# yangyonggit/simple-path-tracer

Measured on AMD Instinct MI355X. Metric: Mrays/sec + Msamples/sec, default scene 1920x1080, 1/2/4/8 MI355X, higher is better.
Workload: dtype f32; 1 GPU; C2: default scene + emitter, 1920x1080, 64 spp, depth 6; scene=default_emitter, width=1920, height=1080, spp=64, max_depth=6, parallelism=tile-sharded x1 (interleaved 32x32 tiles) + RCCL gather to rank 0

## Files before the change

### simple-path-tracer_amd/csrc/kernels_wavefront.hip

```cpp
#include <hip/hip_runtime.h>
#include <hip/hip_ext.h>

#include <algorithm>
#include <cstdlib>
#include <mutex>

#include "cull_prims.h"
#include "sky_split.h"
#include "sptr_internal.h"

#ifndef SPTR_TRACE_WAVES
#define SPTR_TRACE_WAVES 7
#endif
#ifndef SPTR_TRACE_PM_WAVES
#define SPTR_TRACE_PM_WAVES SPTR_TRACE_WAVES
#endif
#ifndef SPTR_TRACE_WP_WAVES
#define SPTR_TRACE_WP_WAVES SPTR_TRACE_WAVES
#endif
#ifndef SPTR_TRACE4_WAVES
#define SPTR_TRACE4_WAVES 7
#endif
#ifndef SPTR_SHADE_WAVES
#define SPTR_SHADE_WAVES 5
// ... 690 lines not shown
  float tn = __builtin_huge_valf();
  uint32_t nxt = 0u, nh = 0u;
#pragma unroll
  for (int k = 0; k < 4; ++k) {
    const bool better = (kAny && kAnyHitFar) ? t[k] > tn : t[k] < tn;
    const bool take = hc[k] & ((kn == 4) | better);
    tn = take ? t[k] : tn;
    kn = take ? k : kn;
    nxt = take ? ln[k] : nxt;
    nh += hc[k] ? 1u : 0u;
  }
  const bool descend = kn < 4;
  if (sp + 3 < N) {
    int pos = sp;
#pragma unroll
    for (int k = 3; k >= 0; --k) {
      stack.lds[pos * kBlock] = ln[k];
      pos += (hc[k] & (k != kn)) ? 1 : 0;
    }
  } else {
    if (sp + (int)nh - 1 > kStack) vc.stack_overflow = 1u;
    int pos = sp;
#pragma unroll
    for (int k = 3; k >= 0; --k)
      if (hc[k] && k != kn && pos < kStack) stack.put(pos++, ln[k]);
  }
  const int spd = sp + (int)nh - 1;
  wk.hit = wk.hit | lhit;
  wk.cur = descend ? nxt : popv;
  wk.sp = descend ? (spd < kStack ? spd : kStack) : ps;
  return (kAny && lhit) || (!descend && sp == 0);
}
template <bool kAny, bool kCount, int N>
__device__ __forceinline__ bool wide_walk_bf(WideWalk& wk, TravStack<N>& stack, const WideNode* nodes,
                                             const uint32_t* prim_ref, const float4* tris, const float4* sph,
                                             const Ray& r, float tnear, float& tfar, uint32_t& ref, Visits& vc, int steps) {
  for (int it = 0; it < steps; ++it)
    if (walk_step_bf<kAny, kCount>(wk, stack, nodes, prim_ref, tris, sph, r, tnear, tfar, ref, vc)) return true;
  return false;
}
template <bool kAny, bool kCount, int kKind = kWalkU, int N>
__device__ __forceinline__ bool wide_walk(WideWalk& wk, TravStack<N>& stack, const WideNode* nodes, const uint4* top,
                                          uint32_t ntop, const uint32_t* prim_ref, const float4* tris, const float4* sph,
                                          const Ray& r, float tnear, float& tfar, uint32_t& ref, Visits& vc, int steps) {
  if constexpr (kKind == kWalkBranchFree)
    return wide_walk_bf<kAny, kCount>(wk, stack, nodes, prim_ref, tris, sph, r, tnear, tfar, ref, vc, steps);
  else if constexpr (kKind == kWalkUnified)
    return wide_walk_u<kAny, kCount>(wk, stack, nodes, top, ntop, prim_ref, tris, sph, r, tnear, tfar, ref, vc, steps);
  else
    return wide_walk_inl<kAny, kCount>(wk, stack, nodes, top, ntop, prim_ref, tris, sph, r, tnear, tfar, ref, vc, steps);
}
template <bool kAny, bool kCount>
__device__ __forceinline__ bool wide_start(WideWalk& wk, uint32_t root, const uint32_t* prim_ref, const float4* tris,
                                           const float4* sph, const Ray& r, float tnear, float& tfar, uint32_t& ref,
                                           Visits& vc) {
  wk.cur = root;
  wk.sp = 0;
  wk.hit = false;
  if (root == kNoHit) return true;
  if (root & kLeafBit) {
    wk.hit = leaf_test<kAny, kCount>(root, prim_ref, tris, sph, r, tnear, tfar, ref, vc);
    return true;
  }
  return false;
}
template <bool kAny, bool kCount, int N>
__device__ __forceinline__ bool traverse_wide(const WideNode* nodes, const uint32_t* prim_ref, const float4* tris,
                                              const float4* sph, uint32_t root, const Ray& r, float tnear, float& tfar,
                                              uint32_t& ref, Visits& vc, LdsStackN<N>& ls) {
  WideWalk wk;
  if (wide_start<kAny, kCount>(wk, root, prim_ref, tris, sph, r, tnear, tfar, ref, vc)) return wk.hit;
  TravStack<N> stack;
  stack.lds = &ls.e[0][threadIdx.x];
  (void)wide_walk<kAny, kCount>(wk, stack, nodes, nullptr, 0u, prim_ref, tris, sph, r, tnear, tfar, ref, vc, 0x7FFFFFFF);
  return wk.hit;
}

struct Staged {
  const BvhNode* nodes;
  const WideNode* nodes4;
  const uint32_t* prim_ref;
  const float4* tris;
  const float4* sph;
};
template <bool kLds>
__device__ __forceinline__ Staged stage_scene(const SceneView& sv, float4* lds) {
  Staged s{sv.nodes, sv.nodes4, sv.prim_ref, sv.tris, sv.sph};
  if (kLds) {
    const bool w4 = sv.width == (uint32_t)kWide;
    const uint32_t nn = (w4 ? sv.num_nodes4 * (uint32_t)sizeof(WideNode) : sv.num_nodes * (uint32_t)sizeof(BvhNode)) / 16u,
                   nt = sv.num_tris * 3u, ns = sv.num_sph;
    const uint32_t np = (sv.num_tris + sv.num_sph + 3u) / 4u;
    const float4* gn = w4 ? reinterpret_cast<const float4*>(sv.nodes4) : reinterpret_cast<const float4*>(sv.nodes);
    const float4* gp = reinterpret_cast<const float4*>(sv.prim_ref);
    for (uint32_t i = threadIdx.x; i < nn; i += blockDim.x) lds[i] = gn[i];
    for (uint32_t i = threadIdx.x; i < nt; i += blockDim.x) lds[nn + i] = sv.tris[i];
    for (uint32_t i = threadIdx.x; i < ns; i += blockDim.x) lds[nn + nt + i] = sv.sph[i];
    for (uint32_t i = threadIdx.x; i < np; i += blockDim.x) lds[nn + nt + ns + i] = gp[i];
    __syncthreads();
    s.nodes = reinterpret_cast<const BvhNode*>(lds);
    s.nodes4 = reinterpret_cast<const WideNode*>(lds);
    s.tris = lds + nn;
    s.sph = lds + nn + nt;
    s.prim_ref = reinterpret_cast<const uint32_t*>(lds + nn + nt + ns);
  }
  return s;
}

__device__ __forceinline__ const uint4* stage_top(const SceneView& sv, float4* dst) {
  const uint32_t n = sv.num_top4 * (uint32_t)(sizeof(WideNode) / 16);
  const uint4* g = reinterpret_cast<const uint4*>(sv.nodes4);
  uint4* d = reinterpret_cast<uint4*>(dst);
  for (uint32_t i = threadIdx.x; i < n; i += blockDim.x) d[i] = g[i];
  return d;
}
__device__ __forceinline__ uint32_t top_lds_offset(const SceneView& sv, bool lds, bool primary, uint32_t nseg) {
  return (lds ? sv.lds_bytes / 16u : 0u) + (primary ? 0u : (4u * (nseg + 1u) + 15u) / 16u);
}

template <bool kW4, bool kAny, bool kCount, int N>
__device__ __forceinline__ bool traverse_w(const Staged& sc, const SceneView& sv, const Ray& r, float tnear, float& tfar,
                                           uint32_t& ref, Visits& vc, LdsStackN<N>& ls) {
  if (kW4) return traverse_wide<kAny, kCount>(sc.nodes4, sc.prim_ref, sc.tris, sc.sph, sv.root4, r, tnear, tfar, ref, vc, ls);
  return traverse<kAny, kCount>(sc.nodes, sc.prim_ref, sc.tris, sc.sph, sv.root, r, tnear, tfar, ref, vc, ls);
}

constexpr uint32_t kEntryFieldBits = 13, kEntryFieldMask = (1u << kEntryFieldBits) - 1u;
template <bool kW4, bool kCount, int N>
__device__ __forceinline__ bool traverse_w_from(const Staged& sc, const SceneView& sv, uint32_t root, const Ray& r,
                                                float& tfar, uint32_t& ref, Visits& vc, LdsStackN<N>& ls) {
  if constexpr (kW4) {
    return traverse_wide<false, kCount>(sc.nodes4, sc.prim_ref, sc.tris, sc.sph, sv.root4, r, 0.0f, tfar, ref, vc, ls);
  } else {
    if (root & kLeafBit) {
      if (root == sv.root) return leaf_test<false, kCount>(root, sc.prim_ref, sc.tris, sc.sph, r, 0.0f, tfar, ref, vc);
      asm volatile("" : "+v"(root));
      const float4* nd = reinterpret_cast<const float4*>(sc.nodes + ((root >> 18) & kEntryFieldMask));
      const uint32_t right = (root >> 17) & 1u;
      const float4 xy = nd[right];
      const float2 z = reinterpret_cast<const float2*>(nd + 2)[right];
      if (kCount) ++vc.nodes;
      float tent;
      if (!slab(xy.x, xy.y, xy.z, xy.w, z.x, z.y, r, 0.0f, tfar, tent)) return false;
      const uint32_t range = kLeafBit | (((root >> 4) & kEntryFieldMask) << kLeafCountBits) | (root & kLeafRangeMask);
      return leaf_test<false, kCount>(range, sc.prim_ref, sc.tris, sc.sph, r, 0.0f, tfar, ref, vc);
    }
    return traverse<false, kCount>(sc.nodes, sc.prim_ref, sc.tris, sc.sph, root, r, 0.0f, tfar, ref, vc, ls);
  }
}

template <bool kW4, bool kAny, bool kCount, int N>
__device__ __forceinline__ bool traverse_w_top(const Staged& sc, const SceneView& sv, const uint4* top, uint32_t ntop,
                                               const Ray& r, float tnear, float& tfar, uint32_t& ref, Visits& vc,
                                               LdsStackN<N>& ls) {
  if constexpr (kW4) {
    WideWalk wk;
    if (wide_start<kAny, kCount>(wk, sv.root4, sc.prim_ref, sc.tris, sc.sph, r, tnear, tfar, ref, vc)) return wk.hit;
    TravStack<N> stack;
    stack.lds = &ls.e[0][threadIdx.x];
    (void)wide_walk<kAny, kCount>(wk, stack, sc.nodes4, top, ntop, sc.prim_ref, sc.tris, sc.sph, r, tnear, tfar, ref, vc,
                                  0x7FFFFFFF);
    return wk.hit;
  }
  return traverse<kAny, kCount>(sc.nodes, sc.prim_ref, sc.tris, sc.sph, sv.root, r, tnear, tfar, ref, vc, ls);
}

__device__ __forceinline__ uint32_t stat_depth(int depth) { return depth < kStatDepths - 1 ? (uint32_t)depth : kStatDepths - 1u; }
__device__ __forceinline__ void hist_ray(uint32_t* s_hist, uint32_t visits) {
  const uint32_t b = visits ? (uint32_t)(32 - __clz(visits)) : 0u;
  atomicAdd(&s_hist[b < (uint32_t)kHistBins ? b : kHistBins - 1u], 1u);
}
__device__ __forceinline__ void hist_init(uint32_t* s_hist) {
  if (threadIdx.x < (uint32_t)kHistBins) s_hist[threadIdx.x] = 0u;
}
__device__ __forceinline__ void hist_flush(const uint32_t* s_hist, unsigned long long* tot, int base) {
  __syncthreads();
  if (threadIdx.x < (uint32_t)kHistBins && s_hist[threadIdx.x]) atomicAdd(&tot[base + threadIdx.x], (unsigned long long)s_hist[threadIdx.x]);
}
__device__ __forceinline__ void flush_depth_nodes(const Visits& vc, unsigned long long* tot, int depth) {
  unsigned long long a = vc.nodes;
  for (int off = 32; off > 0; off >>= 1) a += __shfl_xor(a, off);
  if (lane_id() == 0) atomicAdd(&tot[kTotNodesD + stat_depth(depth)], a);
}

__device__ __forceinline__ void report_stack(const Visits& vc, unsigned long long* tot) {
  if (__ballot(vc.stack_overflow != 0u) && lane_id() == 0u) tot[kTotStackOverflow] = 1ull;
}
// ... 890 lines not shown
        ref = kNoHit;
        if (kCount) v0 = culled ? ~0u : vc.nodes;
        done = walk_start<false, kCount, kW4>(wk, sc, culled ? kNoHit : (kW4 ? sv.root4 : sv.root), r, 0.0f, tfar, ref,
                                              vc);
        have = true;
      }
    }
    if (__ballot(have) == 0ull) {
      if (!more) break;
      continue;
    }
    if (have && !done)
      done = walk_steps<false, kCount, kW4, kKind>(wk, stack, sc, top, ntop, r, 0.0f, tfar, ref, vc,
                                                                          kDynSteps);
    if (!kCount && w.strag_lanes != 0u && drained && (uint32_t)depth < kStragBounces) {
      const unsigned long long act = __ballot(have && !done);
      if (act != 0ull && (uint32_t)__popcll(act) <= w.strag_lanes && have && !done) {
        const uint32_t slot = atomicAdd(&w.work[kWorkStrag + (uint32_t)depth * 32u], 1u);
        if (slot < w.strag_cap) {
          float4* rec = w.strag + ((size_t)depth * w.strag_cap + slot) * kStragRec;
          rec[3] = make_float4(__uint_as_float(wk.cur), __uint_as_float((uint32_t)wk.sp | (wk.hit ? 0x10000u : 0u)),
                               __uint_as_float(ref), tfar);
          uint32_t* st = reinterpret_cast<uint32_t*>(rec + 4);
          for (int q = 0; q < wk.sp; ++q) st[q] = stack.get(q);
          if (kPrimary) {
            Primary pr;
            (void)primary_path(f, idiv, pid, pr);
            rec[0] = f4(f.cam_pos, __uint_as_float(pr.rng));
            rec[1] = f4(r.d, __uint_as_float(pid));
            rec[2] = make_float4(1.0f, 1.0f, 1.0f, __uint_as_float(0u));
          } else {
            rec[0] = rs.o[id];
            rec[1] = rs.d[id];
            rec[2] = f4(xyz(rs.thr[id]), __uint_as_float((uint32_t)depth));
          }
          have = false;
        }
      }
    }
    const bool fin = have && done;
    if (kCount && fin && v0 != ~0u) hist_ray(s_hist, vc.nodes - v0);
    const bool defer = !kPrimary && w.defer_miss != 0u;
    if (fin && !wk.hit) {
      if (defer) {
        if (sh.debug_mode != 1) rs.thr[id] = f4(xyz(rs.thr[id]) * env_color<kCube>(sh, renormalized_again(r.d)), 0.0f);
      } else if (sh.debug_mode == 1) {
        w.rad[pid] = make_float4(0.0f, 0.0f, 0.0f, 0.0f);
      } else {
        const vec3 e = env_color<kCube>(sh, renormalized_again(r.d));
        vec3 rv;
        if (kPrimary) rv = v3(0.0f, 0.0f, 0.0f) + v3(1.0f, 1.0f, 1.0f) * e;
        else rv = xyz(w.rad[pid]) + xyz(rs.thr[id]) * e;
        w.rad[pid] = f4(rv, 0.0f);
      }
    }
    const bool rec = fin && (wk.hit || defer);
    const uint32_t j = block_append(&s_cnt, rec);
    if (kCount) {
      const uint32_t nh = (uint32_t)__popcll(__ballot(fin && wk.hit));
      if (nh && lane_id() == 0u) atomicAdd(&s_hits, nh);
    }
    if (rec) {
      if (seg0 + j < w.hrec_cap) w.hrec.put(seg0 + j, id, wk.hit ? __float_as_uint(tfar) : pid, wk.hit ? ref : kNoHit);
      else w.tot[kTotOverflow] = 1ull;
    }
    if (fin) have = false;
  }
  seg_publish(w.segH, &s_cnt, cap);
  if (kCount && threadIdx.x == 0) atomicAdd(&w.tot[kPrimary ? kTotHitP : kTotHitB], (unsigned long long)s_hits);
  report_stack(vc, w.tot);
  if (kCount) {
    flush_visits(vc, w.tot, kTotNodes);
    if (kPrimary) flush_visits(vc, w.tot, kTotNodesP);
    flush_depth_nodes(vc, w.tot, depth);
    hist_flush(s_hist, w.tot, kTotHistT);
  }
  ktime_end(w);
}

struct Surface {
  vec3 P, n;
  DevMaterial m;
};
__device__ __forceinline__ Surface surface_at(const SceneView& sv, const ShadeView& sh, const DevMaterial* smat,
                                              uint32_t nm, vec3 ro, vec3 rd, float t, uint32_t ref) {
  Surface s;
  s.P = ro + t * rd;
  const uint32_t idx = ref & kIndexMask;
  vec3 ng;
  uint32_t mid;
  if (ref & kSphereBit) {
    const float4 c = sv.sph[idx];
    ng = v3((s.P.x - c.x) / c.w, (s.P.y - c.y) / c.w, (s.P.z - c.z) / c.w);
    mid = sh.geom_mat[sv.sph_geom[idx]];
  } else {
    const float4 c = sv.tris[3 * idx + 2];
    ng = v3(c.y, c.z, c.w);
    mid = sh.tri_mat ? sh.tri_mat[idx] : sh.geom_mat[sv.tri_geom[idx]];
  }
  s.n = safe_normalize(ng);
  if (dot(s.n, rd) > 0.0f) s.n = -s.n;
  s.m = (mid < nm) ? smat[mid] : sh.mats[mid];
  return s;
}

__device__ __forceinline__ void light_at(const DevLight& Lt, vec3 P, vec3& ldir, float& ldist, vec3& Li) {
  if (Lt.type == 0) {
    ldir = v3(Lt.v[0], Lt.v[1], Lt.v[2]);
    ldist = __builtin_huge_valf();
    Li = v3(Lt.radiance[0], Lt.radiance[1], Lt.radiance[2]);
  } else {
    const vec3 lv = v3(Lt.v[0], Lt.v[1], Lt.v[2]) - P;
    ldist = sqrtf(dot(lv, lv));
    ldir = lv / ldist;
    const float att = 1.0f + 0.09f * ldist + 0.032f * ldist * ldist;
    Li = v3(Lt.radiance[0], Lt.radiance[1], Lt.radiance[2]) / att;
  }
}
__device__ __forceinline__ bool light_faces(const DevLight& Lt, const Surface& s) {
  vec3 ldir;
  if (Lt.type == 0) {
    ldir = v3(Lt.v[0], Lt.v[1], Lt.v[2]);
  } else {
    const vec3 lv = v3(Lt.v[0], Lt.v[1], Lt.v[2]) - s.P;
    ldir = lv / sqrtf(dot(lv, lv));
  }
  return fmax_g(dot(s.n, ldir), 0.0f) > 0.0f;
}
__device__ __forceinline__ bool light_term(const DevLight& Lt, const Surface& s, vec3 view, vec3 thr, vec3& so,
                                           vec3& ldir, float& tfar, vec3& contrib) {
  float ldist;
  vec3 Li;
  light_at(Lt, s.P, ldir, ldist, Li);
  const float cs = fmax_g(dot(s.n, ldir), 0.0f);
  if (cs <= 0.0f) return false;
  const float eps = 1e-4f * fmax_g(1.0f, fmax_g(fmax_g(fabsf(s.P.x), fabsf(s.P.y)), fabsf(s.P.z)));
  so = s.P + s.n * eps;
  tfar = ldist - 1e-4f;
  const vec3 fr = eval_brdf(s.m, s.n, view, ldir);
  contrib = thr * (fr * Li * cs);
  return true;
}

__device__ __forceinline__ bool continue_path(const Surface& s, vec3 rd, uint32_t depth, vec3& thr, uint32_t& rng,
                                              vec3& no, vec3& nd) {
  const DevMaterial& m = s.m;
  const vec3 P = s.P, nrm = s.n;
  const vec3 albedo = v3(m.albedo[0], m.albedo[1], m.albedo[2]);
  if (m.metallic > 0.5f) {
    no = P + nrm * 1e-4f;
    nd = safe_renormalize_dir(reflect(rd, nrm));
    thr = thr * (albedo * m.metallic);
    return true;
  }
  if (m.metallic < 0.1f && m.ior > 1.3f) {
    const float ior = m.ior;
    const float cosine = -dot(rd, nrm);
    const float eta = (cosine >= 0.0f) ? (1.0f / ior) : ior;
    const float tr = clamp_g((ior - 1.0f) / 0.7f, 0.0f, 0.95f);
    float r0 = (1.0f - ior) / (1.0f + ior);
    r0 = r0 * r0;
    const float xc = 1.0f - clamp_std(fabsf(cosine), 0.0f, 1.0f);
    const float F = r0 + (1.0f - r0) * xc * xc * xc * xc * xc;
    const float xi = rand01(rng);
    if (xi < F) {
      no = P + nrm * 1e-4f;
      nd = safe_renormalize_dir(reflect(rd, nrm));
      thr = thr * v3(1.0f - tr, 1.0f - tr, 1.0f - tr);
    } else {
      const float ci = -dot(nrm, rd);
      const float kk = 1.0f - eta * eta * (1.0f - ci * ci);
      vec3 refr = v3(0.0f, 0.0f, 0.0f);
      if (!(kk < 0.0f)) refr = eta * rd + (eta * ci - sqrtf(kk)) * nrm;
      if (dot(refr, refr) > 0.0f) {
        no = P - nrm * 1e-4f;
        nd = safe_renormalize_dir(refr);
        thr = thr * v3(tr, tr, tr);
      } else {
        no = P + nrm * 1e-4f;
        nd = safe_renormalize_dir(reflect(rd, nrm));
      }
    }
    return true;
  }
  const float r1 = rand01(rng);
  const float r2 = rand01(rng);
  float sp, cp;
  cosine_sincos(r1, sp, cp);
  const float rr = sqrtf(r2);
  const float lx = rr * cp, ly = rr * sp;
  const float lz = sqrtf(fmax_g(0.0f, 1.0f - r2));
  const vec3 nn = renormalized_again(nrm);
  const vec3 tg = (fabsf(nn.z) < 0.999f) ? normalize_dir(cross(nn, v3(0.0f, 0.0f, 1.0f)))
                                         : normalize_dir(cross(nn, v3(0.0f, 1.0f, 0.0f)));
  const vec3 bt = cross(tg, nn);
  const vec3 sdir = safe_renormalize_dir(tg * lx + bt * ly + nn * lz);
  no = P + nrm * 1e-4f;
  const float surv = fmax_g(fmax_g(albedo.x, albedo.y), albedo.z);
  const float xi = rand01(rng);
  bool cont = true;
  if (depth > 2u) {
    if (xi >= surv) cont = false;
    else thr = thr * (albedo / fmax_g(surv, 1e-6f));
  } else {
    thr = thr * albedo;
  }
  nd = renormalized_again(sdir);
  return cont;
}

__device__ __forceinline__ uint32_t stage_materials(const ShadeView& sh, DevMaterial* smat) {
  const uint32_t nm = sh.num_mats < 32u ? sh.num_mats : 32u;
  for (uint32_t i = threadIdx.x; i < nm * 12u; i += blockDim.x)
    reinterpret_cast<float*>(smat)[i] = reinterpret_cast<const float*>(sh.mats)[i];
  return nm;
}

constexpr int kFuseStack = 6;
template <bool kPrimary, bool kFuse>
__global__ void __launch_bounds__(kBlock, SPTR_SHADE_WAVES)
    k_shade(SceneView sv, ShadeView sh, FrameView fin, WaveView w, int depth, uint32_t nseg_in) {
  const FrameView f = frame_dyn(fin);
  extern __shared__ float4 lds[];
  uint32_t* s_off = reinterpret_cast<uint32_t*>(lds + (kFuse ? sv.lds_bytes / 16u : 0u));
  __shared__ DevMaterial smat[32];
  __shared__ uint32_t s_cnt_n, s_cnt_s, s_rays;
  __shared__ LdsStackN<kFuse ? kFuseStack : 1> s_stack;
  const uint32_t nm = stage_materials(sh, smat);
  if (threadIdx.x == 0) s_cnt_n = s_cnt_s = s_rays = 0u;
  if (blockIdx.x == 0 && threadIdx.x < kXcds) {
    w.work[((uint32_t)depth % 2u) * 256u + threadIdx.x * 32u] = 0u;
    w.work[kWorkTraceQueue + threadIdx.x * 32u] = 0u;
  }
  const Staged sc = stage_scene<kFuse>(sv, lds);
  Visits vc;
  uint32_t rays = 0u;
  uint32_t per_in = 0u;
  const uint32_t n = seg_scan(w.segH, nseg_in, s_off, per_in);

  const RayStream rin = w.rs[depth & 1], rout = w.rs[(depth + 1) & 1];
  const bool last = (uint32_t)(depth + 1) >= f.max_depth;
  const ImageDiv idiv = image_div(f);
  const uint32_t ts = w.tstride, L = w.L;
  const Sched sd = block_sched(n);
  for (uint32_t base = sd.first; base < sd.end; base += sd.step) {
    const uint32_t i = base + threadIdx.x;
    bool active = i < n;
    bool cont = false, shadow = false, dirty = kPrimary;
    uint32_t p = 0u, rng = 0u;
    vec3 rd, thr, radv = v3(0.0f, 0.0f, 0.0f), no, nd;
    Surface sf;
    uint3 h = make_uint3(0u, 0u, 0u);
    if (active) w.hrec.get(seg_slot(s_off, nseg_in, per_in, i), h.x, h.y, h.z);
    if (!kPrimary && active && h.z == kNoHit) {
      p = h.y;
      w.rad[p] = sh.debug_mode == 1 ? make_float4(0.0f, 0.0f, 0.0f, 0.0f) : f4(xyz(w.rad[p]) + xyz(rin.thr[h.x]), 0.0f);
      active = false;
    }
    if (active) {
      vec3 ro;
      if (kPrimary) {
        Primary pr;
        p = h.x;
        primary_path(f, idiv, p, pr);
        ro = f.cam_pos;
        rd = pr.d;
        thr = v3(1.0f, 1.0f, 1.0f);
        rng = pr.rng;
      } else {
        const float4 o4 = rin.o[h.x], d4 = rin.d[h.x];
        ro = xyz(o4);
        rd = xyz(d4);
        thr = xyz(rin.thr[h.x]);
        rng = __float_as_uint(o4.w);
        p = __float_as_uint(d4.w);
      }
      if (sh.debug_mode == 1) {
        radv = v3(1.0f, 1.0f, 1.0f);
        dirty = true;
      } else {
        sf = surface_at(sv, sh, smat, nm, ro, rd, __uint_as_float(h.y), h.z);
        const vec3 emission = v3(sf.m.emission[0], sf.m.emission[1], sf.m.emission[2]);
        if (dot(emission, emission) > 0.0f) {
          if (!kPrimary) radv = xyz(w.rad[p]);
          radv = radv + thr * emission;
          dirty = true;
        }
        for (uint32_t li = 0; li < sh.num_lights; ++li)
          if (light_faces(sh.lights[li], sf)) shadow = true;
      }
    }
    vec3 so, ldir, contrib;
    float stfar = 0.0f;
    bool lit = false;
    if (kFuse) {
      if (shadow) lit = light_term(sh.lights[0], sf, -rd, thr, so, ldir, stfar, contrib);
      shadow = false;
    }
    const uint32_t js = kFuse ? 0u : block_append(&s_cnt_s, shadow);
    if (shadow && sd.seg0 + js >= w.seg_cap) {
      shadow = false;
      w.tot[kTotOverflow] = 1ull;
    }
    const bool carry = !kFuse && (uint32_t)depth == w.carry_depth;
    bool lit0 = false;
    vec3 c0 = v3(0.0f, 0.0f, 0.0f);
    if (shadow) {
      float4* task = w.stask + (size_t)(sd.seg0 + js) * L * ts;
      const vec3 view = -rd;
      for (uint32_t li = 0; li < L; ++li, task += ts) {
        vec3 so, ldir, contrib;
        float tfar;
        if (!light_term(sh.lights[li], sf, view, thr, so, ldir, tfar, contrib)) {
          task[1] = make_float4(0.0f, 0.0f, 0.0f, __uint_as_float(0u));
          continue;
        }
        task[0] = f4(so, tfar);
        if (ts > 2u) task[2] = f4(ldir, 0.0f);
        if (carry) {
          lit0 = true;
          c0 = contrib;
        } else {
          task[1] = f4(contrib, __uint_as_float(p + 1u));
        }
      }
    }
    if (active && sh.debug_mode != 1) cont = continue_path(sf, rd, (uint32_t)depth, thr, rng, no, nd) && !last;
    if (!kFuse && active && dirty) w.rad[p] = f4(radv, 0.0f);
    const uint32_t jn = block_append(&s_cnt_n, cont);
    if (cont && sd.seg0 + jn >= w.seg_cap) {
      cont = false;
      w.tot[kTotOverflow] = 1ull;
    }
    if (lit0) w.stask[(size_t)(sd.seg0 + js) * ts + 1u] = f4(c0, __uint_as_float(cont ? 0u : p + 1u));
    if (cont) {
      rout.o[sd.seg0 + jn] = f4(no, __uint_as_float(rng));
      rout.d[sd.seg0 + jn] = f4(nd, __uint_as_float(p));
      rout.thr[sd.seg0 + jn] = f4(thr, __uint_as_float(lit0 ? sd.seg0 + js + 1u : 0u));
    }
    if (kFuse) {
      if (lit) {
        const Ray r = make_ray(so, ldir);
        uint32_t ref = kNoHit;
        ++rays;
        if (!traverse_w<false, true, false>(sc, sv, r, 1e-4f, stfar, ref, vc, s_stack)) {
          if (!dirty) radv = xyz(w.rad[p]);
          dirty = true;
          radv = radv + contrib;
        }
      }
      if (active && dirty) w.rad[p] = f4(radv, 0.0f);
    }
  }
  if (kFuse) {
    for (int off = 32; off > 0; off >>= 1) rays += __shfl_xor(rays, off);
    if (lane_id() == 0u) atomicAdd(&s_rays, rays);
    report_stack(vc, w.tot);
  }
  __syncthreads();
  if (threadIdx.x == 0) {
    w.segN.cnt[logical_block()] = s_cnt_n;
    w.segS.cnt[logical_block()] = s_cnt_s;
    if (kFuse) w.bstat[blockIdx.x] += s_rays;
    if (blockIdx.x == 0) {
      *w.segN.per = sd.per;
      *w.segS.per = sd.per;
    }
  }
}

template <bool kCube>
__device__ __forceinline__ void bounce_ray(const Staged& sc, const SceneView& sv, const ShadeView& sh, const DevMaterial* smat,
                                           uint32_t nm, const WaveView& w, const RayStream& rin, const RayStream& rout,
                                           int depth, bool last, bool valid, uint32_t id, uint32_t seg0, uint32_t* s_cnt,
                                           Visits& vc, LdsStack& s_stack, uint32_t& rays) {
  bool cont = false, dirty = false, lit = false;
  uint32_t p = 0u, rng = 0u;
  vec3 thr, radv = v3(0.0f, 0.0f, 0.0f), no, nd, so, ldir, contrib;
  float stfar = 0.0f;
  if (valid) {
    const float4 o4 = rin.o[id], d4 = rin.d[id];
    const vec3 ro = xyz(o4), rd = xyz(d4);
    p = __float_as_uint(d4.w);
    rng = __float_as_uint(o4.w);
    thr = xyz(rin.thr[id]);
    float tfar = __builtin_huge_valf();
    uint32_t ref = kNoHit;
    if (!traverse_w<false, false, false>(sc, sv, make_ray(ro, rd), 0.0f, tfar, ref, vc, s_stack)) {
      if (sh.debug_mode == 1) {
        w.rad[p] = make_float4(0.0f, 0.0f, 0.0f, 0.0f);
      } else {
        const vec3 e = env_color<kCube>(sh.env, renormalized_again(rd));
        w.rad[p] = f4(xyz(w.rad[p]) + thr * e, 0.0f);
      }
    } else if (sh.debug_mode == 1) {
      radv = v3(1.0f, 1.0f, 1.0f);
      dirty = true;
    } else {
      const Surface sf = surface_at(sv, sh, smat, nm, ro, rd, tfar, ref);
      const vec3 emission = v3(sf.m.emission[0], sf.m.emission[1], sf.m.emission[2]);
      if (dot(emission, emission) > 0.0f) {
        radv = xyz(w.rad[p]) + thr * emission;
        dirty = true;
      }
      if (light_faces(sh.lights[0], sf)) lit = light_term(sh.lights[0], sf, -rd, thr, so, ldir, stfar, contrib);
      cont = continue_path(sf, rd, (uint32_t)depth, thr, rng, no, nd) && !last;
    }
  }
  const uint32_t jn = block_append(s_cnt, cont);
  if (cont && seg0 + jn >= w.seg_cap) {
    cont = false;
    w.tot[kTotOverflow] = 1ull;
  }
  if (cont) {
    rout.o[seg0 + jn] = f4(no, __uint_as_float(rng));
    rout.d[seg0 + jn] = f4(nd, __uint_as_float(p));
    rout.thr[seg0 + jn] = f4(thr, 0.0f);
  }
  if (lit) {
    uint32_t ref = kNoHit;
    ++rays;
    if (!traverse_w<false, true, false>(sc, sv, make_ray(so, ldir), 1e-4f, stfar, ref, vc, s_stack)) {
      if (!dirty) radv = xyz(w.rad[p]);
      dirty = true;
      radv = radv + contrib;
    }
  }
  if (dirty) w.rad[p] = f4(radv, 0.0f);
}

template <bool kCube, bool kTimed = false>
__global__ void __launch_bounds__(kBlock, SPTR_BOUNCE_WAVES)
    k_bounce(SceneView sv, ShadeView sh, FrameView fin, WaveView w, int depth, uint32_t nseg_in) {
  if constexpr (kTimed) ktime_begin(w);
  const FrameView f = frame_dyn(fin);
  extern __shared__ float4 lds[];
  uint32_t* s_off = reinterpret_cast<uint32_t*>(lds + sv.lds_bytes / 16u);
  __shared__ DevMaterial smat[32];
  __shared__ uint32_t s_cnt_n, s_rays;
  __shared__ LdsStack s_stack;
  const uint32_t nm = stage_materials(sh, smat);
  if (threadIdx.x == 0) s_cnt_n = s_rays = 0u;
  const Staged sc = stage_scene<true>(sv, lds);
  uint32_t per_in = 0u;
  const uint32_t n = seg_scan(w.segN, nseg_in, s_off, per_in);
  if (blockIdx.x == 0 && threadIdx.x == 0) {
    atomicAdd(&w.tot[kTotClosest], (unsigned long long)(n));
    atomicAdd(&w.tot[kTotTracedF], (unsigned long long)(n));
    atomicAdd(&w.tot[kTotTracedD + stat_depth(depth)], (unsigned long long)(n));
  }
  const RayStream rin = w.rs[depth & 1], rout = w.rs[(depth + 1) & 1];
  const bool last = (uint32_t)(depth + 1) >= f.max_depth;
  Visits vc;
  uint32_t rays = 0u;
  const Sched sd = block_sched(n);
  for (uint32_t base = sd.first; base < sd.end; base += sd.step) {
    const uint32_t i = base + threadIdx.x;
    const bool valid = i < n;
    const uint32_t id = valid ? seg_slot(s_off, nseg_in, per_in, i) : 0u;
    bounce_ray<kCube>(sc, sv, sh, smat, nm, w, rin, rout, depth, last, valid, id, sd.seg0, &s_cnt_n, vc, s_stack, rays);
  }
  for (int off = 32; off > 0; off >>= 1) rays += __shfl_xor(rays, off);
  if (lane_id() == 0u) atomicAdd(&s_rays, rays);
  report_stack(vc, w.tot);
  __syncthreads();
  if (threadIdx.x == 0) {
    w.segH.cnt[logical_block()] = s_cnt_n;
    w.bstat[blockIdx.x] += s_rays;
    if (blockIdx.x == 0) *w.segH.per = sd.per;
  }
  if constexpr (kTimed) ktime_end(w);
}

template <bool kCube>
__device__ __forceinline__ void bounce01_path(const Staged& sc, const SceneView& sv, const ShadeView& sh, const DevMaterial* smat,
                                              uint32_t nm, const FrameView& f, const ImageDiv& idiv, const WaveView& w,
                                              const RayStream& rout, bool last1, bool last2, bool valid, uint32_t slot,
                                              uint32_t seg0, uint32_t* s_cnt, Visits& vc, LdsStack& s_stack, uint32_t& rays,
                                              uint32_t& traced) {
  bool cont = false, active = valid;
  uint32_t p = 0u, rng = 0u;
  vec3 thr = v3(1.0f, 1.0f, 1.0f), radv = v3(0.0f, 0.0f, 0.0f), ro, rd;
  if (active) {
    uint3 h;
    w.hrec.get(slot, h.x, h.y, h.z);
    p = h.x;
    Primary pr;
    primary_path(f, idiv, p, pr);
    rng = pr.rng;
    if (sh.debug_mode == 1) {
      radv = v3(1.0f, 1.0f, 1.0f);
      active = false;
    } else {
      const Surface sf = surface_at(sv, sh, smat, nm, f.cam_pos, pr.d, __uint_as_float(h.y), h.z);
      const vec3 emission = v3(sf.m.emission[0], sf.m.emission[1], sf.m.emission[2]);
      if (dot(emission, emission) > 0.0f) radv = radv + thr * emission;
      vec3 so, ldir, contrib;
      float stfar = 0.0f;
      const bool lit = light_faces(sh.lights[0], sf) && light_term(sh.lights[0], sf, -pr.d, thr, so, ldir, stfar, contrib);
      active = continue_path(sf, pr.d, 0u, thr, rng, ro, rd) && !last1;
      if (lit) {
        uint32_t sref = kNoHit;
        ++rays;
        if (!traverse_w<false, true, false>(sc, sv, make_ray(so, ldir), 1e-4f, stfar, sref, vc, s_stack)) radv = radv + contrib;
      }
    }
  }
  bool lit = false;
  vec3 no, nd, so, ldir, contrib;
  float stfar = 0.0f;
  if (active) {
    ++traced;
    float tfar = __builtin_huge_valf();
    uint32_t ref = kNoHit;
    if (!traverse_w<false, false, false>(sc, sv, make_ray(ro, rd), 0.0f, tfar, ref, vc, s_stack)) {
      radv = radv + thr * env_color<kCube>(sh.env, renormalized_again(rd));
    } else {
      const Surface sf = surface_at(sv, sh, smat, nm, ro, rd, tfar, ref);
      const vec3 emission = v3(sf.m.emission[0], sf.m.emission[1], sf.m.emission[2]);
      if (dot(emission, emission) > 0.0f) radv = radv + thr * emission;
      if (light_faces(sh.lights[0], sf)) lit = light_term(sh.lights[0], sf, -rd, thr, so, ldir, stfar, contrib);
      cont = continue_path(sf, rd, 1u, thr, rng, no, nd) && !last2;
    }
  }
  const uint32_t jn = block_append(s_cnt, cont);
  if (cont && seg0 + jn >= w.seg_cap) {
    cont = false;
    w.tot[kTotOverflow] = 1ull;
  }
  if (cont) {
    rout.o[seg0 + jn] = f4(no, __uint_as_float(rng));
    rout.d[seg0 + jn] = f4(nd, __uint_as_float(p));
    rout.thr[seg0 + jn] = f4(thr, 0.0f);
  }
  if (lit) {
    uint32_t sref = kNoHit;
    ++rays;
    if (!traverse_w<false, true, false>(sc, sv, make_ray(so, ldir), 1e-4f, stfar, sref, vc, s_stack)) radv = radv + contrib;
  }
  if (valid) w.rad[p] = f4(radv, 0.0f);
}
#ifndef SPTR_BOUNCE01_WAVES
#define SPTR_BOUNCE01_WAVES 5
#endif
template <bool kCube, bool kTimed = false>
__global__ void __launch_bounds__(kBlock, SPTR_BOUNCE01_WAVES)
    k_bounce01(SceneView sv, ShadeView sh, FrameView fin, WaveView w, uint32_t nseg_in) {
  if constexpr (kTimed) ktime_begin(w);
  const FrameView f = frame_dyn(fin);
  extern __shared__ float4 lds[];
  uint32_t* s_off = reinterpret_cast<uint32_t*>(lds + sv.lds_bytes / 16u);
  __shared__ DevMaterial smat[32];
  __shared__ uint32_t s_cnt_n, s_rays, s_traced;
  __shared__ LdsStack s_stack;
  const uint32_t nm = stage_materials(sh, smat);
  if (threadIdx.x == 0) s_cnt_n = s_rays = s_traced = 0u;
  const Staged sc = stage_scene<true>(sv, lds);
  uint32_t per_in = 0u;
  const uint32_t n = seg_scan(w.segH, nseg_in, s_off, per_in);
  const RayStream rout = w.rs[0];
  const bool last1 = 1u >= f.max_depth, last2 = 2u >= f.max_depth;
  const ImageDiv idiv = image_div(f);
  Visits vc;
  uint32_t rays = 0u, traced = 0u;
  const Sched sd = block_sched(n);
  for (uint32_t base = sd.first; base < sd.end; base += sd.step) {
    const uint32_t i = base + threadIdx.x;
    const bool valid = i < n;
    const uint32_t slot = valid ? seg_slot(s_off, nseg_in, per_in, i) : 0u;
    bounce01_path<kCube>(sc, sv, sh, smat, nm, f, idiv, w, rout, last1, last2, valid, slot, sd.seg0, &s_cnt_n, vc, s_stack, rays,
                         traced);
  }
  for (int off = 32; off > 0; off >>= 1) {
    rays += __shfl_xor(rays, off);
    traced += __shfl_xor(traced, off);
  }
  if (lane_id() == 0u) {
    atomicAdd(&s_rays, rays);
    atomicAdd(&s_traced, traced);
  }
  report_stack(vc, w.tot);
  __syncthreads();
  if (threadIdx.x == 0) {
    w.segN.cnt[logical_block()] = s_cnt_n;
    w.bstat[blockIdx.x] += s_rays;
    if (blockIdx.x == 0) *w.segN.per = sd.per;
    atomicAdd(&w.tot[kTotClosest], (unsigned long long)s_traced);
    atomicAdd(&w.tot[kTotTracedF], (unsigned long long)s_traced);
    atomicAdd(&w.tot[kTotTracedD + 1], (unsigned long long)s_traced);
  }
  if constexpr (kTimed) ktime_end(w);
}

#ifndef SPTR_CHAIN_WAVES
#define SPTR_CHAIN_WAVES 6
#endif
template <bool kCube, bool kTimed = false>
__global__ void __launch_bounds__(kBlock, SPTR_CHAIN_WAVES)
    k_bounce_chain(SceneView sv, ShadeView sh, FrameView fin, WaveView w, int T, uint32_t nseg_in) {
  if constexpr (kTimed) ktime_begin(w);
  const FrameView f = frame_dyn(fin);
  extern __shared__ float4 lds[];
  uint32_t* s_off = reinterpret_cast<uint32_t*>(lds + sv.lds_bytes / 16u);
  __shared__ DevMaterial smat[32];
  __shared__ uint32_t s_cnt[3], s_rays, s_traced;
  __shared__ LdsStack s_stack;
  const uint32_t nm = stage_materials(sh, smat);
  if (threadIdx.x == 0) s_cnt[0] = s_cnt[1] = s_cnt[2] = s_rays = s_traced = 0u;
  const Staged sc = stage_scene<true>(sv, lds);
  uint32_t per_in = 0u;
  const uint32_t n = seg_scan(w.segH, nseg_in, s_off, per_in);
  const bool last1 = 1u >= f.max_depth, last2 = 2u >= f.max_depth;
  const ImageDiv idiv = image_div(f);
  Visits vc;
  uint32_t rays = 0u, traced = 0u;
  const Sched sd = block_sched(n);
  {
    const RayStream rout = w.rs[0];
    for (uint32_t base = sd.first; base < sd.end; base += sd.step) {
      const uint32_t i = base + threadIdx.x;
      const bool valid = i < n;
      const uint32_t slot = valid ? seg_slot(s_off, nseg_in, per_in, i) : 0u;
      bounce01_path<kCube>(sc, sv, sh, smat, nm, f, idiv, w, rout, last1, last2, valid, slot, sd.seg0, &s_cnt[1], vc, s_stack,
                           rays, traced);
    }
  }
  unsigned long long later = 0ull;
  for (int d = 2; d < T; ++d) {
    __syncthreads();
    const uint32_t cnt = s_cnt[(d - 1) % 3];
    if (threadIdx.x == 0) {
      s_cnt[(d + 1) % 3] = 0u;
      if (cnt) atomicAdd(&w.tot[kTotTracedD + stat_depth(d)], (unsigned long long)cnt);
      later += cnt;
    }
    const RayStream rin = w.rs[d & 1], rout = w.rs[(d + 1) & 1];
    const bool last = (uint32_t)(d + 1) >= f.max_depth;
    for (uint32_t j = 0u; j < cnt; j += kBlock) {
      const uint32_t id = sd.seg0 + j + threadIdx.x;
      const bool valid = j + threadIdx.x < cnt && id < w.seg_cap;
      bounce_ray<kCube>(sc, sv, sh, smat, nm, w, rin, rout, d, last, valid, id, sd.seg0, &s_cnt[d % 3], vc, s_stack, rays);
    }
  }
  for (int off = 32; off > 0; off >>= 1) {
    rays += __shfl_xor(rays, off);
    traced += __shfl_xor(traced, off);
  }
  if (lane_id() == 0u) {
    atomicAdd(&s_rays, rays);
    atomicAdd(&s_traced, traced);
  }
  report_stack(vc, w.tot);
  __syncthreads();
  if (threadIdx.x == 0) {
    if ((uint32_t)T < f.max_depth) {
      w.segN.cnt[logical_block()] = s_cnt[(T - 1) % 3];
      if (blockIdx.x == 0) *w.segN.per = sd.per;
    }
    w.bstat[blockIdx.x] += s_rays;
    atomicAdd(&w.tot[kTotClosest], (unsigned long long)s_traced + later);
    atomicAdd(&w.tot[kTotTracedF], (unsigned long long)s_traced + later);
    atomicAdd(&w.tot[kTotTracedD + 1], (unsigned long long)s_traced);
  }
  if constexpr (kTimed) ktime_end(w);
}

#ifndef SPTR_ST_FIRST_WAVES
#define SPTR_ST_FIRST_WAVES 5
#endif
#ifndef SPTR_ST_WAVES
#define SPTR_ST_WAVES 6
#endif
#ifndef SPTR_ST_CLOSE_WAVES
#define SPTR_ST_CLOSE_WAVES 5
#endif
__device__ __forceinline__ void rad_add(const WaveView& w, uint32_t p, bool& dirty, vec3& radv, vec3 c) {
  if (!dirty) radv = xyz(w.rad[p]);
  dirty = true;
  radv = radv + c;
}
__device__ __forceinline__ void shadow_add(const Staged& sc, const SceneView& sv, const WaveView& w, uint32_t p, vec3 so,
                                           vec3 ldir, float stfar, vec3 contrib, bool& dirty, vec3& radv, Visits& vc,
                                           LdsStack& s_stack, uint32_t& rays) {
  uint32_t sref = kNoHit;
  ++rays;
  if (!traverse_w<false, true, false>(sc, sv, make_ray(so, ldir), 1e-4f, stfar, sref, vc, s_stack))
    rad_add(w, p, dirty, radv, contrib);
}
template <bool kCube, bool kFirst, bool kClose>
__device__ __forceinline__ void shade_trace(const Staged& sc, const SceneView& sv, const ShadeView& sh, const DevMaterial* smat,
                                            uint32_t nm, const FrameView& f, const ImageDiv& idiv, const WaveView& w,
                                            const RayStream& rin, const RayStream& rout, int depth, bool last, bool valid,
                                            uint32_t slot, uint32_t seg0, uint32_t* s_cnt, Visits& vc, LdsStack& s_stack,
                                            uint32_t& rays, uint32_t& traced) {
  bool active = false, dirty = kFirst && valid, lit = false;
  uint32_t p = 0u, rng = 0u;
  vec3 thr = v3(1.0f, 1.0f, 1.0f), radv = v3(0.0f, 0.0f, 0.0f), no, nd, so, ldir, contrib;
  float stfar = 0.0f;
  if (valid) {
    vec3 ro, rd;
    float t;
    uint32_t ref;
    if constexpr (kFirst) {
      uint32_t tb;
      w.hrec.get(slot, p, tb, ref);
      t = __uint_as_float(tb);
      Primary pr;
      primary_path(f, idiv, p, pr);
      ro = f.cam_pos;
      rd = pr.d;
      rng = pr.rng;
    } else {
      const float4 o4 = rin.o[slot], d4 = rin.d[slot], t4 = rin.thr[slot];
      ref = rin.ref[slot];
      ro = xyz(o4);
      rd = xyz(d4);
      thr = xyz(t4);
      t = t4.w;
      rng = __float_as_uint(o4.w);
      p = __float_as_uint(d4.w);
    }
    if (sh.debug_mode == 1) {
      radv = v3(1.0f, 1.0f, 1.0f);
      dirty = true;
    } else {
      const Surface sf = surface_at(sv, sh, smat, nm, ro, rd, t, ref);
      const vec3 emission = v3(sf.m.emission[0], sf.m.emission[1], sf.m.emission[2]);
      if (dot(emission, emission) > 0.0f) rad_add(w, p, dirty, radv, thr * emission);
      if (light_faces(sh.lights[0], sf)) lit = light_term(sh.lights[0], sf, -rd, thr, so, ldir, stfar, contrib);
      active = continue_path(sf, rd, (uint32_t)(depth - 1), thr, rng, no, nd);
    }
  }
  if (lit) shadow_add(sc, sv, w, p, so, ldir, stfar, contrib, dirty, radv, vc, s_stack, rays);
  bool hit = false;
  float tfar = __builtin_huge_valf();
  uint32_t href = kNoHit;
  if (active) {
    ++traced;
    hit = traverse_w<false, false, false>(sc, sv, make_ray(no, nd), 0.0f, tfar, href, vc, s_stack);
    if (!hit) rad_add(w, p, dirty, radv, thr * env_color<kCube>(sh.env, renormalized_again(nd)));
  }
  if constexpr (!kClose) {
    const uint32_t jn = block_append(s_cnt, hit);
    if (hit && seg0 + jn >= w.seg_cap) {
      hit = false;
      w.tot[kTotOverflow] = 1ull;
    }
    if (hit) {
      rout.o[seg0 + jn] = f4(no, __uint_as_float(rng));
      rout.d[seg0 + jn] = f4(nd, __uint_as_float(p));
      rout.thr[seg0 + jn] = f4(thr, tfar);
      rout.ref[seg0 + jn] = href;
    }
  } else {
    bool cont = false;
    vec3 no2, nd2;
    lit = false;
    if (hit) {
      const Surface sf = surface_at(sv, sh, smat, nm, no, nd, tfar, href);
      const vec3 emission = v3(sf.m.emission[0], sf.m.emission[1], sf.m.emission[2]);
      if (dot(emission, emission) > 0.0f) rad_add(w, p, dirty, radv, thr * emission);
      if (light_faces(sh.lights[0], sf)) lit = light_term(sh.lights[0], sf, -nd, thr, so, ldir, stfar, contrib);
      if (!last) cont = continue_path(sf, nd, (uint32_t)depth, thr, rng, no2, nd2);
    }
    const uint32_t jn = block_append(s_cnt, cont);
    if (cont && seg0 + jn >= w.seg_cap) {
      cont = false;
      w.tot[kTotOverflow] = 1ull;
    }
    if (cont) {
      rout.o[seg0 + jn] = f4(no2, __uint_as_float(rng));
      rout.d[seg0 + jn] = f4(nd2, __uint_as_float(p));
      rout.thr[seg0 + jn] = f4(thr, 0.0f);
    }
    if (lit) shadow_add(sc, sv, w, p, so, ldir, stfar, contrib, dirty, radv, vc, s_stack, rays);
  }
  if (dirty) w.rad[p] = f4(radv, 0.0f);
}

template <bool kCube, bool kFirst, bool kClose, bool kTimed = false>
__global__ void __launch_bounds__(kBlock, kClose ? SPTR_ST_CLOSE_WAVES : (kFirst ? SPTR_ST_FIRST_WAVES : SPTR_ST_WAVES))
    k_shade_trace(SceneView sv, ShadeView sh, FrameView fin, WaveView w, int depth, uint32_t nseg_in) {
  if constexpr (kTimed) ktime_begin(w);
  const FrameView f = frame_dyn(fin);
  extern __shared__ float4 lds[];
  uint32_t* s_off = reinterpret_cast<uint32_t*>(lds + sv.lds_bytes / 16u);
  __shared__ DevMaterial smat[32];
  __shared__ uint32_t s_cnt_n, s_rays, s_traced;
  __shared__ LdsStack s_stack;
  const uint32_t nm = stage_materials(sh, smat);
  if (threadIdx.x == 0) s_cnt_n = s_rays = s_traced = 0u;
  const Staged sc = stage_scene<true>(sv, lds);
  const SegTable tin = kFirst ? w.segH : w.segN, tout = kFirst ? w.segN : w.segH;
  uint32_t per_in = 0u;
  const uint32_t n = seg_scan(tin, nseg_in, s_off, per_in);
  const RayStream rin = w.rs[depth & 1], rout = w.rs[(depth + 1) & 1];
  const bool last = (uint32_t)(depth + 1) >= f.max_depth;
  const ImageDiv idiv = image_div(f);
  Visits vc;
  uint32_t rays = 0u, traced = 0u;
  const Sched sd = block_sched(n);
  for (uint32_t base = sd.first; base < sd.end; base += sd.step) {
    const uint32_t i = base + threadIdx.x;
    const bool valid = i < n;
    const uint32_t slot = valid ? seg_slot(s_off, nseg_in, per_in, i) : 0u;
    shade_trace<kCube, kFirst, kClose>(sc, sv, sh, smat, nm, f, idiv, w, rin, rout, depth, last, valid, slot, sd.seg0, &s_cnt_n,
                                       vc, s_stack, rays, traced);
  }
  for (int off = 32; off > 0; off >>= 1) {
    rays += __shfl_xor(rays, off);
    traced += __shfl_xor(traced, off);
  }
  if (lane_id() == 0u) {
    atomicAdd(&s_rays, rays);
    atomicAdd(&s_traced, traced);
  }
  report_stack(vc, w.tot);
  __syncthreads();
  if (threadIdx.x == 0) {
    tout.cnt[logical_block()] = s_cnt_n;
    w.bstat[blockIdx.x] += s_rays;
    if (blockIdx.x == 0) *tout.per = sd.per;
    if (s_traced) {
      atomicAdd(&w.tot[kTotClosest], (unsigned long long)s_traced);
      atomicAdd(&w.tot[kTotTracedF], (unsigned long long)s_traced);
      atomicAdd(&w.tot[kTotTracedD + stat_depth(depth)], (unsigned long long)s_traced);
    }
  }
  if constexpr (kTimed) ktime_end(w);
}

template <bool kLds, bool kCount, bool kW4>
__global__ void __launch_bounds__(kBlock, kW4 ? SPTR_SHADOW4_WAVES : SPTR_SHADOW_WAVES) k_shadow(SceneView sv, ShadeView sh, WaveView w, int depth, uint32_t nseg_in) {
  ktime_begin(w);
  __shared__ KernelStack<kLds> s_stack;
  extern __shared__ float4 lds[];
  __shared__ uint32_t s_rays;
  __shared__ uint32_t s_hist[kCount ? kHistBins : 1];
  uint32_t* s_off = reinterpret_cast<uint32_t*>(lds + (kLds ? sv.lds_bytes / 16u : 0u));
  if (threadIdx.x == 0) s_rays = 0u;
  if (kCount) hist_init(s_hist);
  const Staged sc = stage_scene<kLds>(sv, lds);
  uint32_t per_in = 0u;
  const uint32_t n = seg_scan(w.segS, nseg_in, s_off, per_in);
  const uint32_t ts = w.tstride, L = w.L;
  Visits vc;
  uint32_t rays = 0u;
  const Sched sd = block_sched(n);
  for (uint32_t i = sd.first + threadIdx.x; i < sd.end; i += sd.step) {
    const float4* task = w.stask + (size_t)seg_slot(s_off, nseg_in, per_in, i) * L * ts;
    bool any = false;
    uint32_t p = 0u;
    vec3 rv = v3(0.0f, 0.0f, 0.0f);
    for (uint32_t li = 0; li < L; ++li, task += ts) {
      const float4 c = task[1];
      const uint32_t tag = __float_as_uint(c.w);
      if (tag == 0u) continue;
      p = tag - 1u;
      const float4 a = task[0];
      const vec3 dir = (ts > 2u && sh.lights[li].type != 0)
                           ? xyz(task[2])
                           : v3(sh.lights[li].v[0], sh.lights[li].v[1], sh.lights[li].v[2]);
      const Ray r = make_ray(xyz(a), dir);
      float tfar = a.w;
      uint32_t ref = kNoHit;
      ++rays;
      const uint32_t v0 = vc.nodes;
      const bool occ = traverse_w<kW4, true, kCount>(sc, sv, r, 1e-4f, tfar, ref, vc, s_stack);
      if (kCount) hist_ray(s_hist, vc.nodes - v0);
      if (!occ) {
        if (!any) rv = xyz(w.rad[p]);
        any = true;
        rv = rv + xyz(c);
      }
    }
    if (any) w.rad[p] = f4(rv, 0.0f);
  }
  for (int off = 32; off > 0; off >>= 1) rays += __shfl_xor(rays, off);
  if (lane_id() == 0u) atomicAdd(&s_rays, rays);
  __syncthreads();
  if (threadIdx.x == 0) atomicAdd(&w.bstat[blockIdx.x], (unsigned long long)s_rays);
  report_stack(vc, w.tot);
  if (kCount) {
    flush_visits(vc, w.tot, kTotShNodes);
    hist_flush(s_hist, w.tot, kTotHistS);
  }
  ktime_end(w);
}

// ... 15 lines not shown
  const uint32_t n = seg_scan(w.segS, nseg_in, s_off, per_in);
  const uint32_t ts = w.tstride;
  Visits vc;
  uint32_t rays = 0u;
  const Sched sd = block_sched(n);
  const uint32_t nb = block_items(sd, n);
  TravStack<kLdsStackG> stack;
  stack.lds = &s_stack.e[0][threadIdx.x];
  bool have = false, done = false;
  uint32_t p = 0u, ref = kNoHit;
  uint32_t v0 = 0u;
  float tfar = 0.0f;
  vec3 contrib;
  Ray r;
  WideWalk wk;
  XcdQueue xq = xcd_queue(w.work + ((uint32_t)depth % 2u) * 256u, n);
  for (;;) {
    uint32_t item = kNoHit;
    bool more;
    if constexpr (kQueue) {
      item = xcd_take(xq, !have, nullptr, 0u);
      more = !xq.drained;
    } else {
      const uint32_t k = block_take(&s_next, !have);
      if (!have && k < nb) item = block_item(sd, k);
      more = __ballot(!have && k < nb) != 0ull;
    }
    if (item != kNoHit) {
      const float4* task = w.stask + (size_t)seg_slot(s_off, nseg_in, per_in, item) * ts;
      const float4 c = task[1];
      const uint32_t tag = __float_as_uint(c.w);
      if (tag != 0u) {
        p = tag - 1u;
        contrib = xyz(c);
        const float4 a = task[0];
        const vec3 dir = (ts > 2u && sh.lights[0].type != 0) ? xyz(task[2])
                                                            : v3(sh.lights[0].v[0], sh.lights[0].v[1], sh.lights[0].v[2]);
        r = make_ray(xyz(a), dir);
        tfar = a.w;
        ref = kNoHit;
        ++rays;
        if (kCount) v0 = vc.nodes;
        done = wide_start<true, kCount>(wk, sv.root4, sv.prim_ref, sv.tris, sv.sph, r, 1e-4f, tfar, ref, vc);
        have = true;
      }
    }
    if (__ballot(have) == 0ull) {
      if (!more) break;
      continue;
    }
    if (have && !done)
      done = wide_walk<true, kCount, kKind>(wk, stack, sv.nodes4, top, ntop, sv.prim_ref, sv.tris,
                                                                   sv.sph, r, 1e-4f, tfar, ref, vc, kDynSteps);
    if (have && done) {
      if (kCount) hist_ray(s_hist, vc.nodes - v0);
      if (!wk.hit) w.rad[p] = f4(xyz(w.rad[p]) + contrib, 0.0f);
      have = false;
    }
  }
  for (int off = 32; off > 0; off >>= 1) rays += __shfl_xor(rays, off);
  if (lane_id() == 0u) atomicAdd(&s_rays, rays);
  __syncthreads();
  if (threadIdx.x == 0) atomicAdd(&w.bstat[blockIdx.x], (unsigned long long)s_rays);
  report_stack(vc, w.tot);
  if (kCount) {
    flush_visits(vc, w.tot, kTotShNodes);
    hist_flush(s_hist, w.tot, kTotHistS);
  }
  ktime_end(w);
}

template <bool kLds, bool kW4, bool kCube>
__global__ void __launch_bounds__(kBlock, kLds ? SPTR_TAIL_WAVES_LDS : SPTR_TAIL_WAVES) k_tail(SceneView sv, ShadeView sh, FrameView f, WaveView w, int depth0,
                                                 uint32_t nseg_in) {
  __shared__ KernelStack<kLds> s_stack;
  extern __shared__ float4 lds[];
  __shared__ DevMaterial smat[32];
  __shared__ uint32_t s_rays[2], s_next;
  uint32_t* s_off = reinterpret_cast<uint32_t*>(lds + (kLds ? sv.lds_bytes / 16u : 0u));
  const uint32_t nm = stage_materials(sh, smat);
  if (threadIdx.x < 2u) s_rays[threadIdx.x] = 0u;
  if (threadIdx.x == 0u) s_next = 0u;
  const Staged sc = stage_scene<kLds>(sv, lds);
  const uint32_t ntop = (walk_reads_top(kWalkU) && kW4 && !kLds) ? sv.num_top4 : 0u;
  const uint4* top = ntop ? stage_top(sv, lds + top_lds_offset(sv, kLds, false, nseg_in)) : nullptr;
  uint32_t per_in = 0u;
  const uint32_t n = seg_scan(w.segN, nseg_in, s_off, per_in);
  const RayStream rin = w.rs[depth0 & 1];
  const uint32_t L = w.L, D = f.max_depth;
  Visits vc;
  uint32_t n_closest = 0u, n_shadow = 0u;
  const Sched sd = block_sched(n);
  const uint32_t nb = block_items(sd, n);
  bool have = false, loaded = false;
  vec3 ro, rd, thr, radv;
  uint32_t rng = 0u, p = 0u, depth = 0u;
  uint32_t cslot = 0u;
  const bool carried = w.carry_depth != kNoHit && (uint32_t)depth0 == w.carry_depth + 1u;
  for (;;) {
    const uint32_t k = block_take(&s_next, !have);
    if (!have && k < nb) {
      const uint32_t id = seg_slot(s_off, nseg_in, per_in, block_item(sd, k));
      const float4 o4 = rin.o[id], d4 = rin.d[id], t4 = rin.thr[id];
      ro = xyz(o4);
      rd = xyz(d4);
      thr = xyz(t4);
      cslot = carried ? __float_as_uint(t4.w) : 0u;
      rng = __float_as_uint(o4.w);
      p = __float_as_uint(d4.w);
      radv = v3(0.0f, 0.0f, 0.0f);
      loaded = false;
      depth = (uint32_t)depth0;
      have = depth < D;
    }
    if (__ballot(have) == 0ull) break;
    if (!have) continue;
    bool fin = true;
    do {
      if (cslot) {
        const float4* task = w.stask + (size_t)(cslot - 1u) * w.tstride;
        const float4 a = task[0], c = task[1];
        const vec3 sdir = (w.tstride > 2u && sh.lights[0].type != 0) ? xyz(task[2])
                                                                    : v3(sh.lights[0].v[0], sh.lights[0].v[1], sh.lights[0].v[2]);
        ++n_shadow;
        float st = a.w;
        uint32_t sref = kNoHit;
        if (!traverse_w_top<kW4, true, false>(sc, sv, top, ntop, make_ray(xyz(a), sdir), 1e-4f, st, sref, vc, s_stack)) {
          if (!loaded) {
            radv = xyz(w.rad[p]);
            loaded = true;
          }
          radv = radv + xyz(c);
        }
        cslot = 0u;
      }
      ++n_closest;
      float tfar = __builtin_huge_valf();
      uint32_t ref = kNoHit;
      const bool hit = traverse_w_top<kW4, false, false>(sc, sv, top, ntop, make_ray(ro, rd), 0.0f, tfar, ref, vc, s_stack);
      if (sh.debug_mode == 1) {
        radv = hit ? v3(1.0f, 1.0f, 1.0f) : v3(0.0f, 0.0f, 0.0f);
        loaded = true;
        break;
      }
      if (!loaded) {
        radv = xyz(w.rad[p]);
        loaded = true;
      }
      if (!hit) {
        radv = radv + thr * env_color<kCube>(sh.env, renormalized_again(rd));
        break;
      }
      const Surface sf = surface_at(sv, sh, smat, nm, ro, rd, tfar, ref);
      const vec3 emission = v3(sf.m.emission[0], sf.m.emission[1], sf.m.emission[2]);
      if (dot(emission, emission) > 0.0f) radv = radv + thr * emission;
      const vec3 view = -rd;
      for (uint32_t li = 0; li < L; ++li) {
        vec3 so, ldir, contrib;
        float st;
        if (!light_term(sh.lights[li], sf, view, thr, so, ldir, st, contrib)) continue;
        ++n_shadow;
        uint32_t sref = kNoHit;
        if (!traverse_w_top<kW4, true, false>(sc, sv, top, ntop, make_ray(so, ldir), 1e-4f, st, sref, vc, s_stack))
          radv = radv + contrib;
      }
      vec3 no, nd;
      if (!continue_path(sf, rd, depth, thr, rng, no, nd)) break;
      ro = no;
      rd = nd;
      fin = ++depth >= D;
    } while (false);
    if (fin) {
      if (loaded) w.rad[p] = f4(radv, 0.0f);
      have = false;
    }
  }
  for (int off = 32; off > 0; off >>= 1) {
    n_closest += __shfl_xor(n_closest, off);
    n_shadow += __shfl_xor(n_shadow, off);
  }
  if (lane_id() == 0u) {
    atomicAdd(&s_rays[0], n_closest);
    atomicAdd(&s_rays[1], n_shadow);
  }
  __syncthreads();
  if (threadIdx.x == 0) {
    atomicAdd(&w.bstat_closest[blockIdx.x], (unsigned long long)s_rays[0]);
    atomicAdd(&w.bstat[blockIdx.x], (unsigned long long)s_rays[1]);
  }
  report_stack(vc, w.tot);
}

#ifndef SPTR_STRAG_WAVES
#define SPTR_STRAG_WAVES SPTR_TAIL_WAVES
#endif
template <bool kW4, bool kCube>
__global__ void __launch_bounds__(kBlock, SPTR_STRAG_WAVES) k_strag(SceneView sv, ShadeView sh, FrameView f, WaveView w,
                                                                    int depth0) {
  __shared__ KernelStack<false> s_stack;
  __shared__ DevMaterial smat[32];
  __shared__ uint32_t s_rays[2], s_next;
  const uint32_t nm = stage_materials(sh, smat);
  if (threadIdx.x < 2u) s_rays[threadIdx.x] = 0u;
  if (threadIdx.x == 0u) s_next = 0u;
  const Staged sc = stage_scene<false>(sv, nullptr);
  extern __shared__ float4 lds[];
  const uint32_t ntop = walk_reads_top(kWalkU) ? sv.num_top4 : 0u;
  const uint4* top = ntop ? stage_top(sv, lds) : nullptr;
  __syncthreads();
  const uint32_t n = min(w.work[kWorkStrag + (uint32_t)depth0 * 32u], w.strag_cap);
  if (blockIdx.x == 0 && threadIdx.x == 0) atomicAdd(&w.tot[kTotStrag], (unsigned long long)n);
  const float4* in = w.strag + (size_t)depth0 * w.strag_cap * kStragRec;
  TravStack<kLdsStackG> stack;
  stack.lds = &s_stack.e[0][threadIdx.x];
  WideWalk wk;
  float tfar0 = 0.0f;
  uint32_t ref0 = kNoHit;
  const uint32_t L = w.L, D = f.max_depth;
  Visits vc, vr;
  uint32_t n_closest = 0u, n_shadow = 0u;
  const Sched sd = block_sched(n);
  const uint32_t nb = block_items(sd, n);
  bool have = false, loaded = false, first = false;
  vec3 ro, rd, thr, radv;
  uint32_t rng = 0u, p = 0u, depth = 0u;
  for (;;) {
    const uint32_t k = block_take(&s_next, !have);
    if (!have && k < nb) {
      const float4* rec = in + (size_t)block_item(sd, k) * kStragRec;
      const float4 o4 = rec[0], d4 = rec[1], t4 = rec[2], w4 = rec[3];
      wk.cur = __float_as_uint(w4.x);
      wk.sp = (int)(__float_as_uint(w4.y) & 0xFFFFu);
      wk.hit = (__float_as_uint(w4.y) >> 16) != 0u;
      ref0 = __float_as_uint(w4.z);
      tfar0 = w4.w;
      const uint32_t* st = reinterpret_cast<const uint32_t*>(rec + 4);
      for (int q = 0; q < wk.sp; ++q) stack.put(q, st[q]);
      ro = xyz(o4);
      rd = xyz(d4);
      thr = xyz(t4);
      rng = __float_as_uint(o4.w);
      p = __float_as_uint(d4.w);
      depth = __float_as_uint(t4.w);
      loaded = depth == 0u;
      radv = v3(0.0f, 0.0f, 0.0f);
      first = true;
      have = depth < D;
    }
    if (__ballot(have) == 0ull) break;
    if (!have) continue;
    bool fin = true;
    do {
      float tfar = __builtin_huge_valf();
      uint32_t ref = kNoHit;
      bool hit;
      if (first) {
        tfar = tfar0;
        ref = ref0;
        (void)walk_steps<false, true, kW4>(wk, stack, sc, top, ntop, make_ray(ro, rd), 0.0f,
                                                                  tfar, ref, vr, 0x7FFFFFFF);
        hit = wk.hit;
      } else {
        ++n_closest;
        hit = traverse_w_top<kW4, false, false>(sc, sv, top, ntop, make_ray(ro, rd), 0.0f, tfar, ref, vc, s_stack);
      }
      first = false;
      if (sh.debug_mode == 1) {
        radv = hit ? v3(1.0f, 1.0f, 1.0f) : v3(0.0f, 0.0f, 0.0f);
        loaded = true;
        break;
      }
      if (!loaded) {
        radv = xyz(w.rad[p]);
        loaded = true;
      }
      if (!hit) {
        radv = radv + thr * env_color<kCube>(sh.env, renormalized_again(rd));
        break;
      }
      const Surface sf = surface_at(sv, sh, smat, nm, ro, rd, tfar, ref);
      const vec3 emission = v3(sf.m.emission[0], sf.m.emission[1], sf.m.emission[2]);
      if (dot(emission, emission) > 0.0f) radv = radv + thr * emission;
      const vec3 view = -rd;
      for (uint32_t li = 0; li < L; ++li) {
        vec3 so, ldir, contrib;
        float st;
        if (!light_term(sh.lights[li], sf, view, thr, so, ldir, st, contrib)) continue;
        ++n_shadow;
        uint32_t sref = kNoHit;
        if (!traverse_w_top<kW4, true, false>(sc, sv, top, ntop, make_ray(so, ldir), 1e-4f, st, sref, vc, s_stack))
          radv = radv + contrib;
      }
      vec3 no, nd;
      if (!continue_path(sf, rd, depth, thr, rng, no, nd)) break;
      ro = no;
      rd = nd;
      fin = ++depth >= D;
    } while (false);
    if (fin) {
      if (loaded) w.rad[p] = f4(radv, 0.0f);
      have = false;
    }
  }
  for (int off = 32; off > 0; off >>= 1) {
    n_closest += __shfl_xor(n_closest, off);
    n_shadow += __shfl_xor(n_shadow, off);
  }
  if (lane_id() == 0u) {
    atomicAdd(&s_rays[0], n_closest);
    atomicAdd(&s_rays[1], n_shadow);
  }
  __syncthreads();
  if (threadIdx.x == 0) {
    atomicAdd(&w.tot[kTotClosest], (unsigned long long)s_rays[0]);
    atomicAdd(&w.tot[kTotShadow], (unsigned long long)s_rays[1]);
  }
  flush_visits(vr, w.tot, kTotStragNodes);
  report_stack(vc, w.tot);
  report_stack(vr, w.tot);
}

__device__ __forceinline__ bool sky_pixel(const FrameView& f, uint32_t l, int& x, int& y) {
  return pixel_culled(f, l) && local_pixel(f, l, x, y);
}
#ifndef SPTR_SKY_VGPR
#define SPTR_SKY_VGPR 127
#endif
template <bool kCube, bool kCapped, bool kList = false>
__global__ void __launch_bounds__(kBlock) k_sky(EnvView sh, FrameView fin) {
#if SPTR_SKY_VGPR
  if constexpr (kCapped) asm volatile("; k_sky occupancy cap" ::: "v" SPTR_STR(SPTR_SKY_VGPR));
#endif
  const FrameView f = frame_dyn(fin);
  const ImageDiv idiv = image_div(f);
  auto sum_pixel = [&](uint32_t l, int x, int y) {
    vec3 a = v3(0.0f, 0.0f, 0.0f);
    if (!f.reset) a = xyz(f.accum[l]);
    const uint32_t ps = (uint32_t)(y * f.W + x);
    auto sample = [&](uint32_t smp) {
      Primary pr;
      primary_at(f, idiv, x, y, ps, f.acc0 + smp, pr);
      vec3 rv = v3(0.0f, 0.0f, 0.0f);
      if (sh.debug_mode != 1) rv = v3(0.0f, 0.0f, 0.0f) + v3(1.0f, 1.0f, 1.0f) * env_color<kCube>(sh, renormalized_again(pr.d));
      return rv;
    };
    constexpr uint32_t kSkyIlp = SPTR_SKY_ILP;
    uint32_t smp = 0;
    for (; smp + kSkyIlp <= f.k; smp += kSkyIlp) {
      vec3 rv[kSkyIlp];
#pragma unroll
      for (uint32_t j = 0; j < kSkyIlp; ++j) rv[j] = sample(smp + j);
#pragma unroll
      for (uint32_t j = 0; j < kSkyIlp; ++j) a = a + rv[j];
    }
    for (; smp < f.k; ++smp) a = a + sample(smp);
    f.accum[l] = make_float4(a.x, a.y, a.z, __uint_as_float(f.k));
  };
  if constexpr (kList) {
    const SkySplit ss = sky_split(f.plist[f.P], f.plist[f.P + 1u], f.split_threads);
    const uint32_t t = blockIdx.x * blockDim.x + threadIdx.x;
    for (uint32_t l = t; l < f.P; l += grid_threads()) {
      int x, y;
      if (!local_pixel(f, l, x, y)) f.accum[l] = make_float4(0.0f, 0.0f, 0.0f, __uint_as_float(f.k));
// ... 729 lines not shown
  const bool L = sv.lds_bytes != 0;
  const bool P = depth == 0;
  const bool W = sv.width == (uint32_t)kWide;
  const bool cube = sh.env.env != nullptr;
  const unsigned lb = trace_lds(sv, L, P, nseg);
  const EnvView ev = sh.env;
  if (P && L && f.pixel_major == kFoldWave && f.split_threads) {
    return dispatch(
        [&](auto fl) -> unsigned {
          return [&]<bool C, bool Wc, bool Cube, bool T>(Flags<C, Wc, Cube, T>) {
            const unsigned g = resident_grid((const void*)&k_trace_wp<true, C, Wc, Cube, false, T, true, true>, lb);
            SPTR_TIMED_LAUNCH((k_trace_wp<true, C, Wc, Cube, false, T, true, true>), dim3(g), b, lb, s, sv, ev, f, w);
            return g;
          }(fl);
        },
        Flags<>{}, count, W, cube, w.tslot != nullptr);
  }
  if (P && f.pixel_major == kFoldWave) {
    const unsigned g7 = resident_grid((const void*)&k_trace_wp<true, false, false, false>, lb);
    const bool hi = L && !W && (uint64_t)f.P < (uint64_t)g7 * (kBlock / 64u) * 8u * kWpHiOccRounds;
    return dispatch(
        [&](auto fl) -> unsigned {
          return [&]<bool Lc, bool C, bool Wc, bool Cube, bool Hi, bool Ent>(Flags<Lc, C, Wc, Cube, Hi, Ent>) {
            if constexpr (Hi && (Wc || !Lc)) {
              return 0u;
            } else {
              constexpr bool E = Ent || !Hi;
              if (w.tslot) {
                const unsigned g = resident_grid((const void*)&k_trace_wp<Lc, C, Wc, Cube, Hi, true, E>, lb);
                SPTR_TIMED_LAUNCH((k_trace_wp<Lc, C, Wc, Cube, Hi, true, E>), dim3(g), b, lb, s, sv, ev, f, w);
                return g;
              }
              const unsigned g = resident_grid((const void*)&k_trace_wp<Lc, C, Wc, Cube, Hi, false, E>, lb);
              SPTR_TIMED_LAUNCH((k_trace_wp<Lc, C, Wc, Cube, Hi, false, E>), dim3(g), b, lb, s, sv, ev, f, w);
              return g;
            }
          }(fl);
        },
        Flags<>{}, L, count, W, cube, hi, f.entry != nullptr);
  }
  if (P && L && f.pixel_major == kFoldThread) {
    return dispatch(
        [&](auto fl) -> unsigned {
          return [&]<bool C, bool Wc, bool Cube>(Flags<C, Wc, Cube>) {
            const unsigned g = resident_grid((const void*)&k_trace_pm<C, Wc, Cube>, lb);
            SPTR_TIMED_LAUNCH((k_trace_pm<C, Wc, Cube>), dim3(g), b, lb, s, sv, ev, f, w);
            return g;
          }(fl);
        },
        Flags<>{}, count, W, cube);
  }
  if (!L && W) {
    const unsigned lbd = lb + (walk_reads_top(P ? kWalkPrimary : kWalkU) ? sv.num_top4 * (unsigned)sizeof(WideNode) : 0u);
    const bool queue = trace_queue_applies(sv);
    return dispatch(
        [&](auto fl) -> unsigned {
          return [&]<bool C, bool Pc, bool Cube, bool Q>(Flags<C, Pc, Cube, Q>) {
            const unsigned g = resident_grid((const void*)&k_trace_dyn<false, C, Pc, true, Cube, Q>, lbd);
            SPTR_TIMED_LAUNCH((k_trace_dyn<false, C, Pc, true, Cube, Q>), dim3(g), b, lbd, s, sv, ev, f, w, depth, nseg);
            return g;
          }(fl);
        },
        Flags<>{}, count, P, cube, queue);
  }
  return dispatch(
      [&](auto fl) -> unsigned {
        return [&]<bool Lc, bool C, bool Pc, bool Wc, bool Cube>(Flags<Lc, C, Pc, Wc, Cube>) {
          const unsigned g = resident_grid((const void*)&k_trace<Lc, C, Pc, Wc, Cube>, lb);
          SPTR_TIMED_LAUNCH((k_trace<Lc, C, Pc, Wc, Cube>), dim3(g), b, lb, s, sv, ev, f, w, depth, nseg);
          return g;
        }(fl);
      },
      Flags<>{}, L, count, P, W, cube);
}

bool shadow_overlaps(const SceneView& sv, const WaveView& w) {
  return sv.lds_bytes == 0 && sv.width == (uint32_t)kWide && w.L == 1u;
}

bool shade_fuses_shadows(const SceneView& sv, const ShadeView& sh, bool count) {
#ifdef SPTR_EXPERIMENT_KNOBS
  if (getenv("SPTR_NO_FUSE")) return false;
#endif
  return sv.lds_bytes != 0 && sv.width == 2u && sh.num_lights == 1u && !count;
}

unsigned launch_shade(const SceneView& sv, const ShadeView& sh, const FrameView& f, const WaveView& w, int depth,
                      uint32_t nseg, bool fuse, hipStream_t s) {
  const unsigned lb = (fuse ? sv.lds_bytes : 0u) + (4u * (nseg + 1u) + 15u) / 16u * 16u;
  return dispatch(
      [&](auto fl) -> unsigned {
        return [&]<bool Pc, bool Fc>(Flags<Pc, Fc>) {
          const unsigned g = resident_grid((const void*)&k_shade<Pc, Fc>, lb);
          hipLaunchKernelGGL((k_shade<Pc, Fc>), dim3(g), dim3(kBlock), lb, s, sv, sh, f, w, depth, nseg);
          return g;
        }(fl);
      },
      Flags<>{}, depth == 0, fuse);
}

bool cull_entries_apply(const SceneView& sv) { return sv.lds_bytes != 0u && sv.width == 2u; }
uint32_t cull_depth_for(uint32_t spp, bool exact) {
  if (exact) return (uint32_t)kCullEntryDepth;
  return spp >= 16u ? (uint32_t)kCullDepthMax : 4u;
}

void launch_cull(const SceneView& sv, const FrameView& f, uint32_t* mask, uint32_t* plist, uint32_t* entry, bool list_culled,
                 hipStream_t s) {
  if (f.P == 0u) return;
  const uint32_t lc = list_culled ? 1u : 0u;
  if (entry) hipLaunchKernelGGL(k_cull<true>, dim3(f.P / kTilePixels), dim3(kBlock), sv.lds_bytes, s, sv, f, mask, plist, entry, lc);
  else hipLaunchKernelGGL(k_cull<false>, dim3(f.P / kTilePixels), dim3(kBlock), 0, s, sv, f, mask, plist, entry, lc);
}

unsigned launch_bounce(const SceneView& sv, const ShadeView& sh, const FrameView& f, const WaveView& w_in, int depth,
                       uint32_t nseg, bool shade_first, bool close, hipStream_t s) {
  const WaveView w = with_tslot(w_in);
  const unsigned lb = sv.lds_bytes + (4u * (nseg + 1u) + 15u) / 16u * 16u;
  if (!shade_first)
    return dispatch(
        [&](auto fl) -> unsigned {
          return [&]<bool Cube, bool T>(Flags<Cube, T>) {
            const unsigned g = resident_grid((const void*)&k_bounce<Cube, T>, lb);
            SPTR_TIMED_LAUNCH((k_bounce<Cube, T>), dim3(g), dim3(kBlock), lb, s, sv, sh, f, w, depth, nseg);
            return g;
          }(fl);
        },
        Flags<>{}, sh.env.env != nullptr, w.tslot != nullptr);
  return dispatch(
      [&](auto fl) -> unsigned {
        return [&]<bool Cube, bool Cl, bool T>(Flags<Cube, Cl, T>) {
          const unsigned g = resident_grid((const void*)&k_shade_trace<Cube, false, Cl, T>, lb);
          SPTR_TIMED_LAUNCH((k_shade_trace<Cube, false, Cl, T>), dim3(g), dim3(kBlock), lb, s, sv, sh, f, w, depth, nseg);
          return g;
        }(fl);
      },
      Flags<>{}, sh.env.env != nullptr, close, w.tslot != nullptr);
}

unsigned launch_bounce01(const SceneView& sv, const ShadeView& sh, const FrameView& f, const WaveView& w_in, uint32_t nseg,
                         bool shade_first, bool close, hipStream_t s) {
  const WaveView w = with_tslot(w_in);
  const unsigned lb = sv.lds_bytes + (4u * (nseg + 1u) + 15u) / 16u * 16u;
  if (!shade_first)
    return dispatch(
        [&](auto fl) -> unsigned {
          return [&]<bool Cube, bool T>(Flags<Cube, T>) {
            const unsigned g = resident_grid((const void*)&k_bounce01<Cube, T>, lb);
            SPTR_TIMED_LAUNCH((k_bounce01<Cube, T>), dim3(g), dim3(kBlock), lb, s, sv, sh, f, w, nseg);
            return g;
          }(fl);
        },
        Flags<>{}, sh.env.env != nullptr, w.tslot != nullptr);
  return dispatch(
      [&](auto fl) -> unsigned {
        return [&]<bool Cube, bool Cl, bool T>(Flags<Cube, Cl, T>) {
          const unsigned g = resident_grid((const void*)&k_shade_trace<Cube, true, Cl, T>, lb);
          SPTR_TIMED_LAUNCH((k_shade_trace<Cube, true, Cl, T>), dim3(g), dim3(kBlock), lb, s, sv, sh, f, w, 1, nseg);
          return g;
        }(fl);
      },
      Flags<>{}, sh.env.env != nullptr, close, w.tslot != nullptr);
}

unsigned launch_bounce_chain(const SceneView& sv, const ShadeView& sh, const FrameView& f, const WaveView& w_in, int T,
                             uint32_t nseg, hipStream_t s) {
  const WaveView w = with_tslot(w_in);
  const unsigned lb = sv.lds_bytes + (4u * (nseg + 1u) + 15u) / 16u * 16u;
  return dispatch(
      [&](auto fl) -> unsigned {
        return [&]<bool Cube, bool Tm>(Flags<Cube, Tm>) {
          const unsigned g = resident_grid((const void*)&k_bounce_chain<Cube, Tm>, lb);
          SPTR_TIMED_LAUNCH((k_bounce_chain<Cube, Tm>), dim3(g), dim3(kBlock), lb, s, sv, sh, f, w, T, nseg);
          return g;
        }(fl);
      },
      Flags<>{}, sh.env.env != nullptr, w.tslot != nullptr);
}

unsigned launch_shadow(const SceneView& sv, const ShadeView& sh, const WaveView& w_in, int depth, bool count,
                       uint32_t nseg, hipStream_t s) {
  const WaveView w = with_tslot(w_in);
  const dim3 b(kBlock);
  const bool L = sv.lds_bytes != 0;
  const bool W = sv.width == (uint32_t)kWide;
  const unsigned lb = trace_lds(sv, L, false, nseg);
  unsigned g = 0;
  if (!L && W && w.L == 1u) {
    const bool queue = sv.scene_bytes > kL2BytesPerXcd;
    const unsigned lbd = lb + (walk_reads_top(queue ? kWalkU : kWalkInline) ? sv.num_top4 * (unsigned)sizeof(WideNode) : 0u);
    return dispatch(
        [&](auto fl) -> unsigned {
          return [&]<bool C, bool Q>(Flags<C, Q>) {
            const unsigned gq = resident_grid((const void*)&k_shadow_dyn<C, Q>, lbd);
            SPTR_TIMED_LAUNCH((k_shadow_dyn<C, Q>), dim3(gq), b, lbd, s, sv, sh, w, depth, nseg);
            return gq;
          }(fl);
        },
        Flags<>{}, count, queue);
  }
#define SPTR_SHADOW(Lc, C, Wc)                                                                      \
  do {                                                                                              \
    g = resident_grid((const void*)&k_shadow<Lc, C, Wc>, lb);                                       \
    SPTR_TIMED_LAUNCH((k_shadow<Lc, C, Wc>), dim3(g), b, lb, s, sv, sh, w, depth, nseg);           \
  } while (0)
#define SPTR_SHADOW_W(Lc, C) \
  do {                       \
    if (W) SPTR_SHADOW(Lc, C, true); else SPTR_SHADOW(Lc, C, false); \
  } while (0)
  if (L) { if (count) SPTR_SHADOW_W(true, true); else SPTR_SHADOW_W(true, false); }
  else   { if (count) SPTR_SHADOW_W(false, true); else SPTR_SHADOW_W(false, false); }
#undef SPTR_SHADOW_W
#undef SPTR_SHADOW
  return g;
}

unsigned launch_tail(const SceneView& sv, const ShadeView& sh, const FrameView& f, const WaveView& w, int depth0,
                     uint32_t nseg, hipStream_t s) {
  const bool L = sv.lds_bytes != 0;
  const bool W = sv.width == (uint32_t)kWide;
  const unsigned lb = trace_lds(sv, L, false, nseg) + ((walk_reads_top(kWalkU) && !L && W) ? sv.num_top4 * (unsigned)sizeof(WideNode) : 0u);
  return dispatch(
      [&](auto fl) -> unsigned {
        return [&]<bool Lc, bool Wc, bool Cube>(Flags<Lc, Wc, Cube>) {
          const unsigned g = resident_grid((const void*)&k_tail<Lc, Wc, Cube>, lb);
          hipLaunchKernelGGL((k_tail<Lc, Wc, Cube>), dim3(g), dim3(kBlock), lb, s, sv, sh, f, w, depth0, nseg);
          return g;
        }(fl);
      },
      Flags<>{}, L, sv.width == (uint32_t)kWide, sh.env.env != nullptr);
}

bool trace_queue_applies(const SceneView& sv) {
  return sv.lds_bytes == 0u && sv.width == (uint32_t)kWide && sv.scene_bytes > kL2BytesPerXcd;
}
bool strag_applies(const SceneView& sv) { return trace_queue_applies(sv); }
uint32_t hrec_mult(const SceneView& sv) { return trace_queue_applies(sv) ? 2u : 1u; }

#ifndef SPTR_STRAG_GRID
#define SPTR_STRAG_GRID 256
#endif
void launch_strag(const SceneView& sv, const ShadeView& sh, const FrameView& f, const WaveView& w, int depth,
                  hipStream_t s) {
  constexpr unsigned kStragGrid = SPTR_STRAG_GRID;
  const unsigned lb = walk_reads_top(kWalkU) ? sv.num_top4 * (unsigned)sizeof(WideNode) : 0u;
  if (sh.env.env != nullptr) hipLaunchKernelGGL((k_strag<true, true>), dim3(kStragGrid), dim3(kBlock), lb, s, sv, sh, f, w, depth);
  else hipLaunchKernelGGL((k_strag<true, false>), dim3(kStragGrid), dim3(kBlock), lb, s, sv, sh, f, w, depth);
}

void launch_pathtracer(const SceneView& sv, const ShadeView& sh, const FrameView& f, const WaveView& w, hipStream_t s) {
  const bool L = sv.lds_bytes != 0;
// ... 21 lines not shown
          hipLaunchKernelGGL((k_optix<Lc, Wc, Cube>), dim3(g), dim3(kBlock), lb, s, sv, sh, f, w);
          return g;
        }(fl);
      },
      Flags<>{}, L, sv.width == (uint32_t)kWide, sh.env.env != nullptr);
}

void launch_frame_dyn(uint32_t* dyn, uint32_t frame_begin, uint32_t reset, uint32_t total, uint32_t* clear,
                      unsigned long long* t0, hipStream_t s) {
  hipLaunchKernelGGL(k_frame_dyn, dim3(1), dim3(64), 0, s, dyn, frame_begin, reset, total, clear, t0);
}
const void* frame_dyn_kernel() { return (const void*)&k_frame_dyn; }

__global__ void k_spin(uint64_t ticks) {
  const uint64_t t0 = wall_clock64();
  while (wall_clock64() - t0 < ticks) __builtin_amdgcn_s_sleep(8);
}
void launch_spin(uint64_t ticks, hipStream_t s) { hipLaunchKernelGGL(k_spin, dim3(1), dim3(64), 0, s, ticks); }

void launch_sky(const ShadeView& sh, const FrameView& f, bool capped, hipStream_t s) {
#ifdef SPTR_EXPERIMENT_KNOBS
  static const unsigned cap = getenv("SPTR_SKY_BLOCKS") ? (unsigned)atoi(getenv("SPTR_SKY_BLOCKS")) : 16384u;
#else
  constexpr unsigned cap = 16384u;
#endif
  const unsigned g = std::max(1u, std::min<unsigned>((f.P + kBlock - 1u) / kBlock, cap ? cap : 16384u));
  auto go = [&](auto kern) { hipLaunchKernelGGL(kern, dim3(g), dim3(kBlock), 0, s, sh.env, f); };
  if (sh.env.env != nullptr) {
    if (capped) go(k_sky<true, true>); else go(k_sky<true, false>);
  } else {
    if (capped) go(k_sky<false, true>); else go(k_sky<false, false>);
  }
}

void launch_sky_list(const ShadeView& sh, const FrameView& f, hipStream_t s) {
  const unsigned g = std::max(1u, (f.split_threads + kBlock - 1u) / kBlock);
  if (sh.env.env != nullptr) hipLaunchKernelGGL((k_sky<true, false, true>), dim3(g), dim3(kBlock), 0, s, sh.env, f);
  else hipLaunchKernelGGL((k_sky<false, false, true>), dim3(g), dim3(kBlock), 0, s, sh.env, f);
}
uint32_t sky_list_resident_threads(const ShadeView& sh) {
  const unsigned g = sh.env.env != nullptr ? resident_grid((const void*)&k_sky<true, false, true>, 0u)
                                           : resident_grid((const void*)&k_sky<false, false, true>, 0u);
  return g * kBlock;
}

__global__ void __launch_bounds__(kBlock) k_interleave_tiles(const uint4* a, uint32_t na, const uint4* b, uint32_t nb,
                                                             uint4* dst, uint32_t n) {
  constexpr uint32_t kQuads = kTilePixels / 4u;
  for (uint32_t q = blockIdx.x * blockDim.x + threadIdx.x; q < n * kQuads; q += grid_threads()) {
    const uint32_t t = q / kQuads, r = q - t * kQuads, h = t >> 1;
    const uint4* src = (t & 1u) ? b : a;
    const uint32_t ns = (t & 1u) ? nb : na;
    dst[q] = h < ns ? src[h * kQuads + r] : make_uint4(0u, 0u, 0u, 0u);
  }
}
void launch_interleave_tiles(const uint32_t* a, uint32_t na, const uint32_t* b, uint32_t nb, uint32_t* dst,
                             uint32_t n, hipStream_t s) {
  if (n == 0u) return;
  hipLaunchKernelGGL(k_interleave_tiles, dim3(grid_for(n * (kTilePixels / 4u))), dim3(kBlock), 0, s,
                     reinterpret_cast<const uint4*>(a), na, reinterpret_cast<const uint4*>(b), nb,
                     reinterpret_cast<uint4*>(dst), n);
}

void launch_accumulate(const FrameView& f, const WaveView& w_in, float4* accum, uint32_t* tiles, uint8_t* image,
                       bool resolve, hipStream_t s) {
  const WaveView w = with_tslot(w_in);
  if (resolve) hipLaunchKernelGGL(k_accum<true>, dim3(grid_for(f.P)), dim3(kBlock), 0, s, f, w, accum, tiles, image);
  else hipLaunchKernelGGL(k_accum<false>, dim3(grid_for(f.P)), dim3(kBlock), 0, s, f, w, accum, tiles, image);
}

void launch_resolve(const FrameView& f, const float4* accum, uint32_t n, uint32_t* tiles, uint8_t* image,
                    hipStream_t s) {
  hipLaunchKernelGGL(k_resolve, dim3(grid_for(f.P)), dim3(kBlock), 0, s, f, accum, n, tiles, image);
}

__global__ void __launch_bounds__(kBlock) k_tri_materials(const uint32_t* tri_geom, const uint32_t* geom_mat, uint32_t n,
                                                          uint32_t* tri_mat) {
  for (uint32_t i = blockIdx.x * blockDim.x + threadIdx.x; i < n; i += grid_threads()) tri_mat[i] = geom_mat[tri_geom[i]];
}
void launch_tri_materials(const uint32_t* tri_geom, const uint32_t* geom_mat, uint32_t n, uint32_t* tri_mat, hipStream_t s) {
  if (n) hipLaunchKernelGGL(k_tri_materials, dim3(grid_for(n)), dim3(kBlock), 0, s, tri_geom, geom_mat, n, tri_mat);
}

void launch_unpack(const uint32_t* gathered, int G, uint32_t tiles_per_rank, int W, int H, uint8_t* rgb,
                   hipStream_t s) {
  const int ntx = (W + kTile - 1) / kTile;
  hipLaunchKernelGGL(k_unpack, dim3(grid_for((uint64_t)W * H)), dim3(kBlock), 0, s, gathered, G, tiles_per_rank, W,
                     H, ntx, rgb);
}

void launch_query(const SceneView& sv, const uint32_t* tri_orig, const uint32_t* sph_orig, const float* rays, uint32_t n,
                  bool anyhit, uint32_t* ref, float* t, float* ng, uint8_t* occ, uint32_t* stack_overflow, hipStream_t s) {
  hipLaunchKernelGGL(k_query, dim3(grid_for(n)), dim3(kBlock), 0, s, sv, tri_orig, sph_orig, rays, n, anyhit ? 1 : 0,
                     ref, t, ng, occ, stack_overflow);
}

void launch_eval_math(int fn, const float* x, uint32_t n, float* out, hipStream_t s) {
  hipLaunchKernelGGL(k_eval_math, dim3(grid_for(n)), dim3(kBlock), 0, s, fn, x, n, out);
}
void launch_primary(const FrameView& f, float* dirs, uint32_t* rng, hipStream_t s) {
  hipLaunchKernelGGL(k_primary, dim3(grid_for((uint64_t)f.W * f.H)), dim3(kBlock), 0, s, f, dirs, rng);
}

#include "kernels_denoise.h"
#include "kernels_query.h"

}
```

### simple-path-tracer_amd/csrc/sptr_api.cpp

```cpp
#include <hip/hip_runtime.h>

#include <algorithm>
#include <chrono>
#include <cmath>
#include <cstdlib>
#include <cstring>
#include <mutex>
#include <string>
#include <vector>

#include "sptr_internal.h"

#include <dlfcn.h>
#include <execinfo.h>
#include <csignal>
#include <ucontext.h>
#include <unistd.h>

struct sptr_ctx {
  sptr::Context c;
  sptr_ctx* lane = nullptr;
  bool is_lane = false;
  uint32_t lanes_req = 0;
  bool lane_scene = false;
// ... 52 lines not shown
  } dn;
  struct RayQuery {
    sptr::DevBuf keys, index, keys_sorted, order, temp, flag, stage_in, stage_out;
    sptr::DevEvent ev[3];
    bool issued = false;
    bool sorted = false;
    uint32_t count = 0;
  } rq;
  ~sptr_ctx() {
    (void)hipSetDevice(c.device);
    if (c.pending) (void)hipStreamSynchronize(c.pending_stream);
    if (c.stream) (void)hipStreamSynchronize(c.stream);
    if (copy_stream) (void)hipStreamSynchronize(copy_stream);
    if (rq.issued) (void)hipEventSynchronize(rq.ev[2]);
    if (reg_ptr) (void)hipHostUnregister(reg_ptr);
    delete lane;
  }
};

namespace sptr {
namespace {

int fail(Context& c, int code, const std::string& msg) {
  c.err = msg;
  return code;
}
int sync_pending(Context& c);

#define API_HIP(x)                                                                          \
  do {                                                                                      \
    hipError_t e_ = (x);                                                                    \
    if (e_ != hipSuccess) return fail(c, SPTR_ERR_HIP, std::string(#x) + ": " + hipGetErrorString(e_)); \
  } while (0)

inline const Context& shading(const Context& c) { return c.parent ? *c.parent : c; }

constexpr uint64_t kDefaultWavePaths = 1ull << 29;
constexpr double kWaveMemFraction = 0.5;
constexpr uint32_t kSmallBatchTailDepth = 4;
constexpr uint64_t kSmallBatchPaths = 1ull << 25;
uint32_t auto_tail_depth(uint64_t batch_paths, const SceneView& sv) {
  if (sv.lds_bytes == 0u) return sv.scene_bytes <= (4ull << 20) ? 2u : 3u;
  return batch_paths <= kSmallBatchPaths ? kSmallBatchTailDepth : (uint32_t)kMaxDepth;
}
bool bounce_chain_on(const Context& c, uint64_t batch_paths) {
  (void)batch_paths;
  return c.bounce_chain == 2u;
}
#ifndef SPTR_SKY_SPLIT_TNUM
#define SPTR_SKY_SPLIT_TNUM 3
#endif
#ifndef SPTR_SKY_SPLIT_TDIV
#define SPTR_SKY_SPLIT_TDIV 4
#endif
constexpr uint64_t kSkySplitPixelsNum = 5, kSkySplitPixelsDen = 4;
uint32_t sky_split_threads(const Context& c, const SceneView& sv, const ShadeView& sh, const FrameView& fv) {
  uint32_t mode = c.sky_split, threads = c.sky_split_threads;
#ifdef SPTR_EXPERIMENT_KNOBS
  if (const char* e = getenv("SPTR_SKY_SPLIT"); e && mode == 0u && threads == 0u) {
    mode = (uint32_t)atoi(e);
    if (const char* t = strchr(e, ',')) threads = (uint32_t)atoi(t + 1);
  }
#endif
  if (mode == 1u || fv.cull == nullptr || fv.pixel_major != kFoldWave || sv.lds_bytes == 0u) return 0u;
  const uint32_t T = threads ? threads
                             : std::max(1u, sky_list_resident_threads(sh) / (uint32_t)SPTR_SKY_SPLIT_TDIV * (uint32_t)SPTR_SKY_SPLIT_TNUM);
  if (mode == 2u) return T;
  return (uint64_t)fv.P * kSkySplitPixelsDen >= kSkySplitPixelsNum * T ? T : 0u;
}
static bool sky_split_late() {
#ifdef SPTR_EXPERIMENT_KNOBS
  static const bool early = getenv("SPTR_SKY_SPLIT_EARLY") != nullptr;
  return !early;
#else
  return true;
#endif
}
#ifndef SPTR_SHADE_FIRST_MIN_PATHS
#define SPTR_SHADE_FIRST_MIN_PATHS (5ull << 22)
#endif
constexpr uint64_t kShadeFirstMinPaths = SPTR_SHADE_FIRST_MIN_PATHS;
bool shade_first_on(uint64_t batch_paths) { return batch_paths > kShadeFirstMinPaths; }

int resolve_geom_materials(Context& c) {
  const uint32_t nm = (uint32_t)c.mats_host.size();
  const uint32_t ng = c.num_tri_geoms + c.num_sph;
  if (!c.have_scene || nm == 0) return SPTR_OK;
  std::vector<uint32_t> t(ng ? ng : 1, 0u);
  for (uint32_t g = 0; g < ng; ++g) {
    uint32_t m = ~0u;
    if (g < c.geom_material.size() && c.geom_material[g] < nm) m = c.geom_material[g];
    else m = (g < nm) ? g : g % nm;
    t[g] = m;
  }
  API_HIP(c.geom_mat.ensure(t.size() * 4));
  API_HIP(hipMemcpy(c.geom_mat.p, t.data(), t.size() * 4, hipMemcpyHostToDevice));
#ifndef SPTR_TRI_MAT
#define SPTR_TRI_MAT 1
#endif
  c.tri_mat.release();
  if (SPTR_TRI_MAT && scene_view(c).lds_bytes == 0u && c.num_tri_refs) {
    API_HIP(c.tri_mat.ensure((size_t)c.num_tri_refs * 4));
    launch_tri_materials(static_cast<const uint32_t*>(c.tri_geom.p), static_cast<const uint32_t*>(c.geom_mat.p),
                         c.num_tri_refs, static_cast<uint32_t*>(c.tri_mat.p), c.stream);
    API_HIP(hipGetLastError());
    API_HIP(hipStreamSynchronize(c.stream));
  }
  return SPTR_OK;
}

inline bool host_local_pixel(const Context& c, uint32_t l, int& x, int& y) {
  return shard_pixel(c.W, c.H, c.G, c.R, l, x, y);
}

size_t seg_table_bytes() { return 3 * (kMaxSegs + 4) * 4 + 2 * kMaxSegs * 8 + kWorkWords * 4; }

uint64_t wave_path_bytes(uint32_t L, uint32_t ts, uint32_t hrec_mult) {
  return 2 * (3 * 16 + 4) + hrec_mult * kHitBytes + 16 + (uint64_t)L * ts * 16;
}
uint64_t wave_slack_bytes(uint32_t L, uint32_t ts, uint32_t k_slack, uint32_t hrec_mult) {
  const uint64_t recs = (uint64_t)kMaxSegs * kBlock;
  return recs * (2 * (3 * 16 + 4) + (uint64_t)(L ? L : 1u) * ts * 16) + hrec_mult * recs * k_slack * kHitBytes;
}

int ensure_wave(Context& c, uint64_t cap, uint32_t L, uint32_t ts, uint32_t k_slack, uint32_t hrec_mult) {
  WaveBufs& b = c.wb;
  L = L ? L : 1u;
  const size_t hrec_bytes = ((size_t)cap + (size_t)kMaxSegs * kBlock * k_slack) * kHitBytes * hrec_mult;
  const bool grow = b.hrec.bytes < hrec_bytes || !(b.cap >= cap && b.L * b.ts >= L * ts && b.rad.p) || !b.seg.p;
  if (grow && sync_pending(c) != SPTR_OK) return SPTR_ERR_HIP;
  if (grow) ++c.epoch;
  if (!b.seg.p) {
    API_HIP(b.seg.ensure(seg_table_bytes()));
    API_HIP(hipMemset(b.seg.p, 0, seg_table_bytes()));
  }
  if (strag_applies(scene_view(c))) API_HIP(b.strag.ensure((size_t)kStragHandoffBounces * kStragCap * kStragRec * 16u));
  API_HIP(b.hrec.ensure(hrec_bytes));
  if (b.cap >= cap && b.L * b.ts >= L * ts && b.rad.p) return SPTR_OK;
  const size_t n = (size_t)cap, ns = n + (size_t)kMaxSegs * kBlock;
  for (auto& r : b.rs)
    for (DevBuf& x : r) API_HIP(x.ensure(ns * 16));
  for (DevBuf& x : b.rs_ref) API_HIP(x.ensure(ns * 4));
  API_HIP(b.rad.ensure(n * 16));
  API_HIP(b.stask.ensure(ns * L * ts * 16));
  b.cap = cap;
  b.L = L;
  b.ts = ts;
  return SPTR_OK;
}

uint32_t task_stride(const Context& c) {
  for (const DevLight& l : shading(c).lights_host)
    if (l.type != 0) return 3u;
  return 2u;
}

WaveView wave_view(Context& c) {
  const WaveBufs& wb = c.wb;
  WaveView w;
  for (int b = 0; b < 2; ++b) {
    w.rs[b].o = static_cast<float4*>(wb.rs[b][0].p);
    w.rs[b].d = static_cast<float4*>(wb.rs[b][1].p);
    w.rs[b].thr = static_cast<float4*>(wb.rs[b][2].p);
    w.rs[b].ref = static_cast<uint32_t*>(wb.rs_ref[b].p);
  }
  const uint64_t hcap = std::min<uint64_t>(wb.hrec.bytes / kHitBytes, 0xFFFFFFFFull);
  w.hrec.tr = static_cast<uint2*>(wb.hrec.p);
  w.hrec.id = reinterpret_cast<uint32_t*>(static_cast<char*>(wb.hrec.p) + hcap * 8u);
  w.rad = static_cast<float4*>(wb.rad.p);
  w.stask = static_cast<float4*>(wb.stask.p);
  uint32_t* seg = static_cast<uint32_t*>(wb.seg.p);
  w.segN = SegTable{seg, seg + kMaxSegs};
  w.segH = SegTable{seg + (kMaxSegs + 4), seg + (kMaxSegs + 4) + kMaxSegs};
  w.segS = SegTable{seg + 2 * (kMaxSegs + 4), seg + 2 * (kMaxSegs + 4) + kMaxSegs};
  w.bstat = reinterpret_cast<unsigned long long*>(seg + 3 * (kMaxSegs + 4));
  w.bstat_closest = w.bstat + kMaxSegs;
  w.work = reinterpret_cast<uint32_t*>(w.bstat_closest + kMaxSegs);
  w.tot = static_cast<unsigned long long*>(c.w_tot.p);
  w.L = (uint32_t)shading(c).lights_host.size();
  w.tstride = task_stride(c);
  w.defer_miss = 0u;
  w.seg_cap = (uint32_t)(wb.cap + (uint64_t)kMaxSegs * kBlock);
  w.hrec_cap = (uint32_t)hcap;
  w.strag = static_cast<float4*>(wb.strag.p);
  w.strag_cap = wb.strag.p ? kStragCap : 0u;
  w.strag_lanes = 0u;
  w.carry_depth = kNoHit;
  return w;
}

FrameView frame_view(const Context& c, const sptr_frame& f) {
  FrameView v;
  v.W = f.width;
  v.H = f.height;
  v.ntx = (f.width + kTile - 1) / kTile;
  v.G = c.G;
  v.R = c.R;
  v.P = c.P;
  v.k = 1;
  v.acc0 = f.frame_begin;
  v.max_depth = f.max_depth;
  v.div_P = make_fastdiv(c.P ? c.P : 1u);
  v.div_ntx = make_fastdiv((uint32_t)v.ntx);
  v.valid = 0;
  {
    const int ntx = (c.W + kTile - 1) / kTile;
    for (uint32_t lt = 0; lt < c.local_tiles; ++lt) {
      const uint32_t t = lt * (uint32_t)c.G + (uint32_t)c.R;
      const int x0 = (int)(t % (uint32_t)ntx) * kTile, y0 = (int)(t / (uint32_t)ntx) * kTile;
      v.valid += (uint32_t)(std::min(kTile, c.W - x0) * std::min(kTile, c.H - y0));
    }
  }
  const sptr_camera& k = f.camera;
  v.cam_pos = v3(k.pos[0], k.pos[1], k.pos[2]);
  v.cam_f = v3(k.forward[0], k.forward[1], k.forward[2]);
  v.cam_r = v3(k.right[0], k.right[1], k.right[2]);
  v.cam_u = v3(k.up[0], k.up[1], k.up[2]);
  v.half_w = k.half_width;
  v.half_h = k.half_height;
#ifdef SPTR_EXPERIMENT_KNOBS
  static const uint32_t ablate = getenv("SPTR_ABLATE") ? (uint32_t)atoi(getenv("SPTR_ABLATE")) : 0u;
  v.ablate = ablate;
#else
  v.ablate = 0u;
#endif
  v.accum = static_cast<float4*>(c.accum.p);
  v.reset = 0;
  v.pixel_major = 0;
  v.dyn = nullptr;
  v.cull = nullptr;
  v.cull_depth = 4u;
  v.sky_fold = 0u;
  v.plist = nullptr;
  v.unculled = nullptr;
  v.entry = nullptr;
  v.split_threads = 0u;
  v.integrator = f.integrator;
  v.spf = f.samples_per_frame ? f.samples_per_frame : 4u;
  return v;
}

ShadeView shade_view(const Context& cc) {
  const Context& c = shading(cc);
  ShadeView s{};
  s.mats = static_cast<const DevMaterial*>(c.mats.p);
  s.num_mats = (uint32_t)c.mats_host.size();
  s.geom_mat = static_cast<const uint32_t*>(c.geom_mat.p);
  s.tri_mat = cc.parent ? nullptr : static_cast<const uint32_t*>(c.tri_mat.p);
  s.num_lights = (uint32_t)c.lights_host.size();
  for (uint32_t i = 0; i < s.num_lights; ++i) s.lights[i] = c.lights_host[i];
  s.env.env = static_cast<const float4*>(c.env.p);
  s.env.env_size = c.env_size;
  s.env.env_intensity = c.env_intensity;
  s.env.env_clamp = c.env_clamp;
  s.env.debug_mode = c.debug_mode;
  s.debug_mode = c.debug_mode;
  return s;
}

constexpr int kStages = 10;
#ifndef SPTR_CALL_SPAN
#define SPTR_CALL_SPAN 1
#endif
struct StageTimer {
  Context& c;
  bool on;
  bool trace_only;
  hipStream_t s;
  hipError_t err = hipSuccess;
  std::string what;
  size_t open = SIZE_MAX;
  size_t call = SIZE_MAX;
  size_t alloc() {
    if (c.events_used == c.events.size()) {
      DevEvent e;
      const hipError_t r = hipEventCreate(e.put());
      if (r != hipSuccess) {
        if (err == hipSuccess) {
          err = r;
          what = "stage event create";
        }
        return SIZE_MAX;
      }
      c.events.push_back(std::move(e));
    }
    return c.events_used++;
  }
  bool capturing = false;
  size_t next() {
    const size_t i = alloc();
    if (i != SIZE_MAX && err == hipSuccess) {
      err = hipEventRecord(c.events[i], s);
      if (err != hipSuccess) what = "stage event record";
    }
    return i;
  }
  static bool one_launch(int stage) { return stage == 1 || stage == 5 || stage == 9 || stage == 3; }
  bool launch_timed = false;
  bool quiet = false, quiet_open = false;
  void begin(int stage) {
    if (quiet && !on && !capturing && one_launch(stage)) {
      g_launch_timing = LaunchTiming{c.quiet_ev[0], c.quiet_ev[1]};
      quiet_open = true;
      return;
    }
    if (!on || capturing || (trace_only && !one_launch(stage))) return;
    if (one_launch(stage) && (c.time_by_events || stage == 3)) {
      const size_t b = alloc(), e = alloc();
      if (b == SIZE_MAX || e == SIZE_MAX) return;
      open = c.marks.size();
      c.marks.push_back(StageMark{stage, b, e});
      g_launch_timing = LaunchTiming{c.events[b], c.events[e]};
      launch_timed = true;
      return;
    }
    if (one_launch(stage)) {
      if (!c.tslots.p || c.tslots_used >= kTimeSlots) return;
      open = c.marks.size();
      c.marks.push_back(StageMark{stage, SIZE_MAX, SIZE_MAX, c.tslots_used});
      g_tslot = static_cast<unsigned long long*>(c.tslots.p) + (size_t)kTimeSlotWords * c.tslots_used++;
      launch_timed = true;
      return;
    }
    open = c.marks.size();
    c.marks.push_back(StageMark{stage, next(), SIZE_MAX});
  }
  void end() {
    if (quiet_open) {
      quiet_open = false;
      g_launch_timing = LaunchTiming{};
      return;
// ... 809 lines not shown
    x->lane->is_lane = true;
    if (hipEventCreateWithFlags(x->lane_fork.put(), hipEventDisableTiming) != hipSuccess ||
        hipEventCreateWithFlags(x->lane_join.put(), hipEventDisableTiming) != hipSuccess) {
      (void)sptr_destroy(x);
      *out = nullptr;
      return SPTR_ERR_HIP;
    }
  }
  return SPTR_OK;
}

static int create_one(int device, sptr_ctx** out, const sptr_ctx* parent) {
  if (!out) return SPTR_ERR_INVALID;
  install_segv_trace();
  *out = nullptr;
  int n = 0;
  if (hipGetDeviceCount(&n) != hipSuccess || n <= 0) return SPTR_ERR_NO_DEVICE;
  if (device < 0 || device >= n) return SPTR_ERR_INVALID;
  sptr_ctx* x = new sptr_ctx();
  Context& c = x->c;
  c.device = device;
  if (parent) {
    c.parent = &parent->c;
    c.prio_lo = parent->c.prio_lo;
    c.prio_hi = parent->c.prio_hi;
    if (hipSetDevice(device) != hipSuccess || !create_events(c)) {
      delete x;
      return SPTR_ERR_HIP;
    }
  } else if (hipSetDevice(device) != hipSuccess || hipStreamCreateWithFlags(c.stream.put(), hipStreamNonBlocking) != hipSuccess ||
      hipStreamCreateWithFlags(c.cap_stream.put(), hipStreamNonBlocking) != hipSuccess ||
      hipDeviceGetStreamPriorityRange(&c.prio_lo, &c.prio_hi) != hipSuccess ||
      hipStreamCreateWithPriority(c.side_stream.put(), hipStreamNonBlocking, c.prio_lo) != hipSuccess ||
      hipStreamCreateWithPriority(c.cap_side.put(), hipStreamNonBlocking, c.prio_lo) != hipSuccess ||
      hipStreamCreateWithPriority(c.side2_stream.put(), hipStreamNonBlocking, c.prio_lo) != hipSuccess ||
      hipStreamCreateWithPriority(c.cap_side2.put(), hipStreamNonBlocking, c.prio_lo) != hipSuccess ||
      !create_events(c)) {
    delete x;
    return SPTR_ERR_HIP;
  }
  int khz = 0;
  if (c.wb.seg.ensure(seg_table_bytes()) != hipSuccess || c.w_tot.ensure(kTotWords * 8) != hipSuccess ||
      c.dyn.ensure(kDynBytes) != hipSuccess || hipMemset(c.wb.seg.p, 0, seg_table_bytes()) != hipSuccess ||
      c.tslots.ensure((size_t)kTimeSlots * kTimeSlotWords * 8) != hipSuccess ||
      hipMemset(c.tslots.p, 0, (size_t)kTimeSlots * kTimeSlotWords * 8) != hipSuccess ||
      hipDeviceGetAttribute(&khz, hipDeviceAttributeWallClockRate, device) != hipSuccess || khz <= 0) {
    delete x;
    return SPTR_ERR_OOM;
  }
  c.wall_khz = khz;
  *out = x;
  return SPTR_OK;
}

int sptr_destroy(sptr_ctx* x) {
  if (!x) return SPTR_ERR_INVALID;
  delete x;
  return SPTR_OK;
}

const char* sptr_last_error(const sptr_ctx* x) { return x ? x->c.err.c_str() : "null context"; }

static int set_debug_mode_one(sptr_ctx* x, int mode) {
  if (!x) return SPTR_ERR_INVALID;
  x->c.debug_mode = mode;
  ++x->c.epoch;
  return SPTR_OK;
}

static int set_leaf_size_one(sptr_ctx* x, uint32_t n) {
  if (!x) return SPTR_ERR_INVALID;
  if (n > kMaxLeafSize) return fail(x->c, SPTR_ERR_INVALID, "leaf size must be 0 (automatic) or 1..16");
  x->c.leaf_size = n;
  ++x->c.epoch;
  return SPTR_OK;
}

static int set_bvh_width_one(sptr_ctx* x, uint32_t width) {
  if (!x) return SPTR_ERR_INVALID;
  if (width != 0 && width != 2 && width != (uint32_t)kWide)
    return fail(x->c, SPTR_ERR_INVALID, "bvh width must be 0 (auto), 2 or " + std::to_string(kWide));
  x->c.bvh_width = width;
  ++x->c.epoch;
  return SPTR_OK;
}

static int set_tail_depth_one(sptr_ctx* x, uint32_t depth) {
  if (!x) return SPTR_ERR_INVALID;
  if (depth > (uint32_t)kMaxDepth) return fail(x->c, SPTR_ERR_INVALID, "tail depth must be 0 (automatic) or 1..32");
  x->c.tail_depth = depth;
  ++x->c.epoch;
  return SPTR_OK;
}

static int set_bounce_chain_one(sptr_ctx* x, uint32_t mode) {
  if (!x) return SPTR_ERR_INVALID;
  if (mode > 2u) return fail(x->c, SPTR_ERR_INVALID, "bounce chain must be 0 (automatic), 1 (off) or 2 (on)");
  x->c.bounce_chain = mode;
  return SPTR_OK;
}

static int set_sky_split_one(sptr_ctx* x, uint32_t mode, uint32_t bulk_threads) {
  if (!x) return SPTR_ERR_INVALID;
  if (mode > 2u) return fail(x->c, SPTR_ERR_INVALID, "sky split must be 0 (automatic), 1 (off) or 2 (on)");
  x->c.sky_split = mode;
  x->c.sky_split_threads = bulk_threads;
  return SPTR_OK;
}

static int set_split_refs_one(sptr_ctx* x, uint32_t max_pieces) {
  if (!x) return SPTR_ERR_INVALID;
  if (max_pieces == 0u) max_pieces = 1u;
  if (max_pieces > 32u || (max_pieces & (max_pieces - 1u)))
    return fail(x->c, SPTR_ERR_INVALID, "split references: 0 (default: 1, none) or a power of two up to 32");
  x->c.split_pieces = max_pieces;
  ++x->c.epoch;
  return SPTR_OK;
}

static int set_stragglers_one(sptr_ctx* x, uint32_t lanes) {
  if (!x) return SPTR_ERR_INVALID;
  if (lanes > 64u) return fail(x->c, SPTR_ERR_INVALID, "straggler lanes: 0 (no hand-off) to 64");
  x->c.strag_lanes = lanes;
  ++x->c.epoch;
  return SPTR_OK;
}

static int set_wave_paths_one(sptr_ctx* x, uint64_t max_paths) {
  if (!x) return SPTR_ERR_INVALID;
  if (max_paths > (1ull << 30)) return fail(x->c, SPTR_ERR_INVALID, "wave paths above 2^30");
  x->c.wave_paths = max_paths;
  ++x->c.epoch;
  return SPTR_OK;
}

static int upload_scene_one(sptr_ctx* x, const sptr_scene* s) {
  if (!x || !s) return SPTR_ERR_INVALID;
  Context& c = x->c;
  if (sync_pending(c) != SPTR_OK) return SPTR_ERR_HIP;
  API_HIP(hipSetDevice(c.device));
  if ((s->num_tris && (!s->indices || !s->positions || !s->tri_geom_first)) || (s->num_spheres && !s->spheres) ||
      ((s->num_tri_geoms + s->num_spheres) && !s->geom_material))
    return fail(c, SPTR_ERR_INVALID, "scene: null array with nonzero count");
  if ((uint64_t)s->num_tris + s->num_spheres >= (1ull << (31 - kLeafCountBits)))
    return fail(c, SPTR_ERR_INVALID, "scene too large (at most 2^26 primitives)");
  if (s->num_tri_geoms && s->tri_geom_first[s->num_tri_geoms] != s->num_tris)
    return fail(c, SPTR_ERR_INVALID, "scene: tri_geom_first must end at num_tris");
  for (uint64_t i = 0; i < (uint64_t)s->num_tris * 3; ++i)
    if (s->indices[i] >= s->num_verts) return fail(c, SPTR_ERR_INVALID, "scene: vertex index out of range");
  std::vector<uint32_t> tg(s->num_tris);
  for (uint32_t g = 0; g < s->num_tri_geoms; ++g) {
    if (s->tri_geom_first[g] > s->tri_geom_first[g + 1]) return fail(c, SPTR_ERR_INVALID, "scene: geom offsets");
    for (uint32_t i = s->tri_geom_first[g]; i < s->tri_geom_first[g + 1]; ++i) tg[i] = g;
  }
  c.have_scene = false;
  c.num_tri_geoms = s->num_tri_geoms;
  c.geom_first.assign(s->tri_geom_first, s->tri_geom_first + (s->num_tri_geoms ? s->num_tri_geoms + 1 : 0));
  c.geom_material.assign(s->geom_material, s->geom_material + s->num_tri_geoms + s->num_spheres);
  const int rc = build_lbvh(c, s->positions, s->num_verts, s->indices, s->num_tris, s->spheres, s->num_spheres, tg.data(),
                            s->num_tri_geoms);
  if (rc != SPTR_OK) return rc;
  c.have_scene = true;
  ++c.epoch;
  return resolve_geom_materials(c);
}

int sptr_scene_info(const sptr_ctx* x, uint32_t* num_prims, uint32_t* num_nodes, uint32_t* depth, double* build_ms) {
  if (!x) return SPTR_ERR_INVALID;
  const Context& c = x->c;
  if (num_prims) *num_prims = c.num_tris + c.num_sph;
  if (num_nodes) *num_nodes = c.num_nodes;
  if (depth) *depth = c.bvh_depth;
  if (build_ms) *build_ms = c.build_ms;
  return SPTR_OK;
}

int sptr_scene_layout_info(const sptr_ctx* x, sptr_scene_layout* out) {
  if (!x || !out) return SPTR_ERR_INVALID;
  const Context& c = x->c;
  const SceneView sv = scene_view(c);
  out->num_tris = c.num_tris;
  out->num_spheres = c.num_sph;
  out->num_nodes = c.num_nodes;
  out->leaf_size = c.leaf_used;
  out->bvh_depth = c.bvh_depth;
  out->lds_bytes = sv.lds_bytes;
  out->bvh_width = sv.width;
  out->num_nodes = sv.width == (uint32_t)kWide ? c.num_nodes4 : c.num_nodes;
  out->node_bytes = sv.width == (uint32_t)kWide ? (uint64_t)c.num_nodes4 * sizeof(WideNode) : (uint64_t)c.num_nodes * sizeof(BvhNode);
  out->tri_bytes = (uint64_t)c.num_tri_refs * 48u;
  out->sphere_bytes = (uint64_t)c.num_sph * 16u;
  out->prim_ref_bytes = ((uint64_t)c.num_tri_refs + c.num_sph) * 4u;
  out->num_prim_refs = c.num_tri_refs + c.num_sph;
  return SPTR_OK;
}

static int set_materials_one(sptr_ctx* x, const sptr_material* m, uint32_t n) {
  if (!x || (n && !m)) return SPTR_ERR_INVALID;
  Context& c = x->c;
  if (sync_pending(c) != SPTR_OK) return SPTR_ERR_HIP;
  if (n == 0) return fail(c, SPTR_ERR_INVALID, "at least one material is required");
  API_HIP(hipSetDevice(c.device));
  c.mats_host.resize(n);
  std::memcpy(c.mats_host.data(), m, sizeof(DevMaterial) * n);
  API_HIP(c.mats.ensure(sizeof(DevMaterial) * n));
  API_HIP(hipMemcpy(c.mats.p, c.mats_host.data(), sizeof(DevMaterial) * n, hipMemcpyHostToDevice));
  ++c.epoch;
  return resolve_geom_materials(c);
}

static int set_lights_one(sptr_ctx* x, const sptr_light* l, uint32_t n) {
  if (!x || (n && !l)) return SPTR_ERR_INVALID;
  Context& c = x->c;
  if (n > (uint32_t)kMaxLights) return fail(c, SPTR_ERR_INVALID, "too many lights");
  c.lights_host.resize(n);
  ++c.epoch;
  for (uint32_t i = 0; i < n; ++i) {
    DevLight& d = c.lights_host[i];
    d.type = l[i].type;
    if (l[i].type == 0) {
      const vec3 v = normalize(-v3(l[i].v[0], l[i].v[1], l[i].v[2]));
      d.v[0] = v.x; d.v[1] = v.y; d.v[2] = v.z;
    } else if (l[i].type == 1) {
      d.v[0] = l[i].v[0]; d.v[1] = l[i].v[1]; d.v[2] = l[i].v[2];
    } else {
      return fail(c, SPTR_ERR_INVALID, "unknown light type");
    }
    const vec3 r = v3(l[i].color[0], l[i].color[1], l[i].color[2]) * l[i].intensity;
    d.radiance[0] = r.x; d.radiance[1] = r.y; d.radiance[2] = r.z;
    d.pad = 0.0f;
  }
  return SPTR_OK;
}

static int set_environment_one(sptr_ctx* x, const sptr_environment* e) {
  if (!x) return SPTR_ERR_INVALID;
  Context& c = x->c;
  if (sync_pending(c) != SPTR_OK) return SPTR_ERR_HIP;
// ... 627 lines not shown
  uint32_t *vi = nullptr, *vo = nullptr;
  char* tmp = nullptr;
  size_t tb = 0;
  API_HIP(radix_sort_pairs_u64(nullptr, tb, nullptr, nullptr, nullptr, nullptr, n, c.stream));
  API_HIP(d.alloc(&ki, n));
  API_HIP(d.alloc(&ko, n));
  API_HIP(d.alloc(&vi, n));
  API_HIP(d.alloc(&vo, n));
  API_HIP(d.alloc(&tmp, tb));
  if (n) {
    API_HIP(hipMemcpy(ki, keys, (size_t)n * 8, hipMemcpyHostToDevice));
    API_HIP(hipMemcpy(vi, vals, (size_t)n * 4, hipMemcpyHostToDevice));
  }
  API_HIP(radix_sort_pairs_u64(tmp, tb, ki, ko, vi, vo, n, c.stream));
  API_HIP(hipStreamSynchronize(c.stream));
  if (n) {
    API_HIP(hipMemcpy(keys_out, ko, (size_t)n * 8, hipMemcpyDeviceToHost));
    API_HIP(hipMemcpy(vals_out, vo, (size_t)n * 4, hipMemcpyDeviceToHost));
  }
  return SPTR_OK;
}

int sptr_eval_math(sptr_ctx* x, int fn, const float* in, uint32_t n, float* out) {
  if (!x || !out || (fn != SPTR_MATH_COSINE_SINCOS && fn != SPTR_MATH_GAMMA) || (fn == SPTR_MATH_GAMMA && n && !in))
    return SPTR_ERR_INVALID;
  Context& c = x->c;
  if (sync_pending(c) != SPTR_OK) return SPTR_ERR_HIP;
  API_HIP(hipSetDevice(c.device));
  const uint32_t m = fn == SPTR_MATH_COSINE_SINCOS ? (1u << 24) : n;
  const size_t out_n = fn == SPTR_MATH_COSINE_SINCOS ? 2u * (size_t)m : (size_t)m;
  DevTemps d;
  float *di = nullptr, *dout = nullptr;
  API_HIP(d.alloc(&di, fn == SPTR_MATH_GAMMA ? (size_t)n : 4));
  API_HIP(d.alloc(&dout, out_n));
  if (fn == SPTR_MATH_GAMMA && n) API_HIP(hipMemcpy(di, in, (size_t)n * 4, hipMemcpyHostToDevice));
  if (m) launch_eval_math(fn, di, m, dout, c.stream);
  API_HIP(hipGetLastError());
  API_HIP(hipStreamSynchronize(c.stream));
  if (out_n) API_HIP(hipMemcpy(out, dout, out_n * 4, hipMemcpyDeviceToHost));
  return SPTR_OK;
}

int sptr_scan_u32(sptr_ctx* x, const uint32_t* in, uint32_t n, uint32_t* out) {
  if (!x || (n && (!in || !out))) return SPTR_ERR_INVALID;
  Context& c = x->c;
  if (sync_pending(c) != SPTR_OK) return SPTR_ERR_HIP;
  API_HIP(hipSetDevice(c.device));
  DevTemps d;
  uint32_t *di = nullptr, *dout = nullptr;
  char* tmp = nullptr;
  size_t tb = 0;
  API_HIP(scan_u32(nullptr, tb, nullptr, nullptr, n, c.stream));
  API_HIP(d.alloc(&di, n));
  API_HIP(d.alloc(&dout, n));
  API_HIP(d.alloc(&tmp, tb));
  if (n) API_HIP(hipMemcpy(di, in, (size_t)n * 4, hipMemcpyHostToDevice));
  API_HIP(scan_u32(tmp, tb, di, dout, n, c.stream));
  API_HIP(hipStreamSynchronize(c.stream));
  if (n) API_HIP(hipMemcpy(out, dout, (size_t)n * 4, hipMemcpyDeviceToHost));
  return SPTR_OK;
}


static int lane_forward(sptr_ctx* x, int rc_lane) {
  if (!x || !x->lane || rc_lane == SPTR_OK) return SPTR_OK;
  return fail(x->c, rc_lane, std::string("pixel lane: ") + x->lane->c.err);
}

int sptr_upload_scene(sptr_ctx* x, const sptr_scene* s) {
  const int rc = upload_scene_one(x, s);
  if (rc != SPTR_OK) return rc;
  x->geom_first_valid = false;
  x->dn.snap_valid = false;
  if (x->split) x->c.W = 0;
  x->split = false;
  x->lane_scene = false;
  if (x->lane && scene_view(x->c).lds_bytes != 0) {
    Context& cy = x->lane->c;
    if (!cy.stream && hipStreamCreateWithPriority(cy.stream.put(), hipStreamNonBlocking, x->c.prio_lo) != hipSuccess)
      return fail(x->c, SPTR_ERR_HIP, "pixel lane: stream creation failed");
    const int r1 = upload_scene_one(x->lane, s);
    if (r1 != SPTR_OK) return lane_forward(x, r1);
    x->lane_scene = true;
  }
  return SPTR_OK;
}

int sptr_set_dynamic(sptr_ctx* x, uint32_t on) {
  if (!x) return SPTR_ERR_INVALID;
  x->c.dynamic = on != 0u;
  x->c.dynamic_xf = (on & SPTR_DYNAMIC_TRANSFORMS) != 0u;
  if (x->lane) x->lane->c.dynamic = x->c.dynamic;
  return SPTR_OK;
}

static int refit_one(Context& c, const float* d_pos, const float* d_sph, const float* d_xf) {
  if (sync_pending(c) != SPTR_OK) return SPTR_ERR_HIP;
  const int rc = refit_lbvh(c, d_pos, reinterpret_cast<const float4*>(d_sph), d_xf);
  ++c.epoch;
  return rc;
}

static int refit_scene(sptr_ctx* x, const char* who, const float* d_pos, const float* d_sph, const float* d_xf,
                       std::chrono::steady_clock::time_point t0) {
  Context& c = x->c;
  auto& d = x->dn;
  if (d.motion_on && d.last.valid && d.last.gen == d.geom_gen) {
    const int rs = refit_snapshot(c);
    if (rs != SPTR_OK) return rs;
    d.snap_gen = d.geom_gen;
    d.snap_valid = true;
  }
  const uint64_t epoch_before = c.epoch;
  const int rc = refit_one(c, d_pos, d_sph, d_xf);
  ++d.geom_gen;
  if (rc != SPTR_OK) return rc;
  if (d.motion_on)
    for (sptr_ctx::Denoise::Pass* p : {&d.last, &d.carry})
      if (p->valid && p->epoch == epoch_before) p->epoch = c.epoch;
  if (x->lane && x->lane_scene) {
    Context& cy = x->lane->c;
    if (!cy.rf.valid) return fail(c, SPTR_ERR_INVALID, std::string(who) + ": the pixel lane's scene is not dynamic");
    const int r1 = refit_one(cy, d_pos, d_sph, d_xf);
    if (r1 != SPTR_OK) return lane_forward(x, r1);
  }
  c.rf.ms_wall = std::chrono::duration<double, std::milli>(std::chrono::steady_clock::now() - t0).count();
  return SPTR_OK;
}

int sptr_update_geometry(sptr_ctx* x, const float* positions, uint32_t num_verts, const float* spheres,
                         uint32_t num_spheres, uint32_t flags) {
  if (!x) return SPTR_ERR_INVALID;
  Context& c = x->c;
  if (x->is_lane) return fail(c, SPTR_ERR_INVALID, "update_geometry: not on a lane context");
  if (!c.have_scene) return fail(c, SPTR_ERR_NO_SCENE, "update_geometry: no scene uploaded");
  if (c.rf.split)
    return fail(c, SPTR_ERR_INVALID, "update_geometry: the scene was built with split references (sptr_set_split_refs)");
  if (!c.rf.valid) return fail(c, SPTR_ERR_INVALID, "update_geometry: the scene was not uploaded with sptr_set_dynamic(1)");
  if (!positions && !spheres) return fail(c, SPTR_ERR_INVALID, "update_geometry: no coordinates given");
  if ((positions && num_verts != c.rf.num_verts) || (spheres && num_spheres != c.num_sph))
    return fail(c, SPTR_ERR_INVALID, "update_geometry: counts differ from the uploaded scene's");
  if (flags & ~(uint32_t)SPTR_UPDATE_DEVICE_PTRS) return fail(c, SPTR_ERR_INVALID, "update_geometry: unknown flags");
  const auto t0 = std::chrono::steady_clock::now();
  API_HIP(hipSetDevice(c.device));
  if (sync_pending(c) != SPTR_OK) return SPTR_ERR_HIP;
  const float *d_pos = positions, *d_sph = spheres;
  if (!(flags & SPTR_UPDATE_DEVICE_PTRS)) {
    if (positions) {
      API_HIP(c.rf.in_pos.ensure((size_t)num_verts * 12));
      API_HIP(hipMemcpyAsync(c.rf.in_pos.p, positions, (size_t)num_verts * 12, hipMemcpyHostToDevice, c.stream));
      d_pos = static_cast<const float*>(c.rf.in_pos.p);
    }
    if (spheres) {
      API_HIP(c.rf.in_sph.ensure((size_t)num_spheres * 16));
      API_HIP(hipMemcpyAsync(c.rf.in_sph.p, spheres, (size_t)num_spheres * 16, hipMemcpyHostToDevice, c.stream));
      d_sph = static_cast<const float*>(c.rf.in_sph.p);
    }
  }
  return refit_scene(x, "update_geometry", d_pos, d_sph, nullptr, t0);
}

static int transforms_ready(sptr_ctx* x, const char* who) {
  Context& c = x->c;
  const std::string w(who);
  if (x->is_lane) return fail(c, SPTR_ERR_INVALID, w + ": not on a lane context");
  if (!c.have_scene) return fail(c, SPTR_ERR_NO_SCENE, w + ": no scene uploaded");
// ... 639 lines not shown
  Context& c = x->c;
  auto& d = x->dn;
  if (x->is_lane) return fail(c, SPTR_ERR_INVALID, "read_motion: not on a lane context");
  if (!d.ran || !d.hist_ran || !d.motion_used)
    return fail(c, SPTR_ERR_INVALID, "read_motion: the last render call ran no pass on the motion path (sptr_set_history_motion)");
  API_HIP(hipSetDevice(c.device));
  if (sync_pending(c) != SPTR_OK) return SPTR_ERR_HIP;
  API_HIP(hipMemcpy(out, d.motion.p, (size_t)d.last_W * d.last_H * 8, hipMemcpyDeviceToHost));
  return SPTR_OK;
}

int sptr_motion_info(sptr_ctx* x, uint32_t* snapshots, double* ms_snapshot, uint32_t* used) {
  if (!x) return SPTR_ERR_INVALID;
  Context& c = x->c;
  if (x->is_lane) return fail(c, SPTR_ERR_INVALID, "motion_info: not on a lane context");
  const auto& d = x->dn;
  if (snapshots) *snapshots = c.rf.snapshots;
  if (ms_snapshot) *ms_snapshot = c.rf.ms_snapshot;
  if (used) *used = d.ran && d.hist_ran && d.motion_used ? 1u : 0u;
  return SPTR_OK;
}

static int lane_shading_sync(sptr_ctx* x) {
  if (!x || !x->lane || x->lane->c.pending == 0) return SPTR_OK;
  if (sync_pending(x->lane->c) != SPTR_OK) return fail(x->c, SPTR_ERR_HIP, std::string("pixel lane: ") + x->lane->c.err);
  return SPTR_OK;
}
static int lane_shading_changed(sptr_ctx* x, int rc) {
  if (x && x->lane) ++x->lane->c.epoch;
  return rc;
}

int sptr_set_debug_mode(sptr_ctx* x, int mode) { return lane_shading_changed(x, set_debug_mode_one(x, mode)); }

int sptr_set_leaf_size(sptr_ctx* x, uint32_t n) {
  const int rc = set_leaf_size_one(x, n);
  return rc == SPTR_OK ? lane_forward(x, set_leaf_size_one(x ? x->lane : nullptr, n)) : rc;
}

int sptr_set_bvh_width(sptr_ctx* x, uint32_t width) {
  const int rc = set_bvh_width_one(x, width);
  return rc == SPTR_OK ? lane_forward(x, set_bvh_width_one(x ? x->lane : nullptr, width)) : rc;
}

int sptr_set_tail_depth(sptr_ctx* x, uint32_t depth) {
  const int rc = set_tail_depth_one(x, depth);
  return rc == SPTR_OK ? lane_forward(x, set_tail_depth_one(x ? x->lane : nullptr, depth)) : rc;
}

int sptr_set_bounce_chain(sptr_ctx* x, uint32_t mode) {
  const int rc = set_bounce_chain_one(x, mode);
  return rc == SPTR_OK ? lane_forward(x, set_bounce_chain_one(x ? x->lane : nullptr, mode)) : rc;
}

int sptr_set_sky_split(sptr_ctx* x, uint32_t mode, uint32_t bulk_threads) {
  const int rc = set_sky_split_one(x, mode, bulk_threads);
  return rc == SPTR_OK ? lane_forward(x, set_sky_split_one(x ? x->lane : nullptr, mode, bulk_threads)) : rc;
}

int sptr_sky_split_info(sptr_ctx* x, uint32_t* bulk_threads) {
  if (!x || !bulk_threads) return SPTR_ERR_INVALID;
  *bulk_threads = x->c.sky_split_last;
  return SPTR_OK;
}

int sptr_set_split_refs(sptr_ctx* x, uint32_t max_pieces) {
  const int rc = set_split_refs_one(x, max_pieces);
  return rc == SPTR_OK ? lane_forward(x, set_split_refs_one(x ? x->lane : nullptr, max_pieces)) : rc;
}

int sptr_set_stragglers(sptr_ctx* x, uint32_t lanes) {
  const int rc = set_stragglers_one(x, lanes);
  return rc == SPTR_OK ? lane_forward(x, set_stragglers_one(x ? x->lane : nullptr, lanes)) : rc;
}

int sptr_set_wave_paths(sptr_ctx* x, uint64_t max_paths) {
  const int rc = set_wave_paths_one(x, max_paths);
  return rc == SPTR_OK ? lane_forward(x, set_wave_paths_one(x ? x->lane : nullptr, max_paths)) : rc;
}

int sptr_set_materials(sptr_ctx* x, const sptr_material* m, uint32_t n) {
  const int rs = lane_shading_sync(x);
  if (rs != SPTR_OK) return rs;
  return lane_shading_changed(x, set_materials_one(x, m, n));
}

int sptr_set_lights(sptr_ctx* x, const sptr_light* l, uint32_t n) {
  return lane_shading_changed(x, set_lights_one(x, l, n));
}

int sptr_set_environment(sptr_ctx* x, const sptr_environment* e) {
  const int rs = lane_shading_sync(x);
  if (rs != SPTR_OK) return rs;
  return lane_shading_changed(x, set_environment_one(x, e));
}

int sptr_set_launch_mode(sptr_ctx* x, uint32_t mode) {
  const int rc = set_launch_mode_one(x, mode);
  return rc == SPTR_OK ? lane_forward(x, set_launch_mode_one(x->lane, mode)) : rc;
}

}
```

### simple-path-tracer_amd/csrc/sptr_internal.h

```cpp
#pragma once
#include <hip/hip_runtime.h>

#include <string>
#include <utility>
#include <vector>

#include "dev_owned.h"
#include "sptr_hip.h"
#include "sptr_math.h"
#include "tile_map.h"

namespace sptr {

constexpr uint32_t kLeafBit = 0x80000000u;
constexpr uint32_t kSphereBit = 0x40000000u;
constexpr uint32_t kIndexMask = 0x3FFFFFFFu;
constexpr uint32_t kLeafCountBits = 5;
constexpr uint32_t kLeafRangeMask = 0xFu;
constexpr uint32_t kLeafDirect = 0x10u;
constexpr uint32_t kLeafDirectSphere = 0x08u;
constexpr uint32_t kLeafCountMask = (1u << kLeafCountBits) - 1u;
constexpr uint32_t kMaxLeafSize = kLeafRangeMask + 1u;
constexpr uint32_t kNoHit = 0xFFFFFFFFu;
constexpr int kTile = 32;
constexpr int kTilePixels = kTile * kTile;
constexpr int kMaxLights = 8;
constexpr int kWide = 4;
constexpr int kWideLevels = 2;
constexpr int kQWords = 1;
constexpr int kTopLevels = 3;
constexpr int kMaxDepth = 32;
constexpr int kStack = 96;
constexpr int kBlock = 256;
#ifndef SPTR_TREELET_PASSES
#define SPTR_TREELET_PASSES 3
#endif
constexpr uint32_t kLdsSceneBytes = 48 * 1024;

struct BvhNode {
  float4 lxy;
  float4 rxy;
  float4 z;
  uint4 link;
};
static_assert(sizeof(BvhNode) == 64, "node size");

struct alignas(16) WideNode {
  float ox, oy, oz;
  uint32_t ex;
  uint32_t link[kWide];
  uint32_t q[6][kQWords];
  uint32_t parent;
  uint32_t pad[1];
};
static_assert(sizeof(WideNode) == 64, "node size");

struct DevMaterial {
  float albedo[3];
  float metallic;
  float roughness;
  float emission[3];
  float ior;
  int32_t type;
  float pad[2];
};
static_assert(sizeof(DevMaterial) == 48, "material size");

struct DevLight {
  int32_t type;
  float v[3];
  float radiance[3];
  float pad;
};

struct SceneView {
  const BvhNode* nodes;
  const WideNode* nodes4;
  const uint32_t* prim_ref;
  const float4* tris;
  const float4* sph;
  const uint32_t* tri_geom;
  const uint32_t* sph_geom;
  uint32_t num_nodes, num_tris, num_sph, root;
  uint32_t num_nodes4, root4;
  uint32_t num_top4;
  uint32_t width;
  uint32_t lds_bytes;
  uint64_t scene_bytes;
};

struct EnvView {
  const float4* env;
  int32_t env_size;
  float env_intensity, env_clamp;
  int32_t debug_mode;
};

struct ShadeView {
  const DevMaterial* mats;
  uint32_t num_mats;
  const uint32_t* geom_mat;
  const uint32_t* tri_mat;
  uint32_t num_lights;
  DevLight lights[kMaxLights];
  EnvView env;
  int32_t debug_mode;
};

struct FrameView {
  int32_t W, H, ntx, G, R;
  FastDiv div_P, div_ntx;
  uint32_t P;
  uint32_t k;
  uint32_t acc0;
  uint32_t max_depth;
  uint32_t valid;
  vec3 cam_pos, cam_f, cam_r, cam_u;
  float half_w, half_h;
  uint32_t ablate;
  float4* accum;
  uint32_t reset;
  uint32_t split_threads;
  const uint32_t* dyn;
  uint32_t pixel_major;
  uint32_t integrator;
  uint32_t spf;
  vec3 ox_u, ox_v, ox_w;
  vec3 ox_light_dir, ox_light_rad;
  uint32_t ox_has_light;
  const uint32_t* cull;
  uint32_t sky_fold;
  uint32_t cull_depth;
  const uint32_t* plist;
  const uint32_t* unculled;
  const uint32_t* entry;
};
static_assert(sizeof(FrameView) == 272, "FrameView: split_threads sits in padding, the kernels' arguments keep their layout");
constexpr size_t kDynBytes = 2048;

enum : uint32_t { kFoldNone = 0, kFoldThread = 1, kFoldWave = 2 };

constexpr uint32_t kWorkTraceQueue = 512;
constexpr uint32_t kWorkStrag = 768;
constexpr uint32_t kStragBounces = 4;
constexpr uint32_t kWorkWords = kWorkStrag + 32u * kStragBounces;
constexpr uint32_t kStragCap = 1u << 17;
constexpr uint32_t kStragRec = 4u + (uint32_t)kStack / 4u;
static_assert(kStragRec * 4u - 16u >= (uint32_t)kStack, "a straggler record holds the whole traversal stack");
constexpr uint32_t kStragLanesDefault = 12;
#ifndef SPTR_STRAG_MAXD
#define SPTR_STRAG_MAXD 1
#endif
constexpr uint32_t kStragHandoffBounces = SPTR_STRAG_MAXD;
constexpr uint32_t kMaxSegs = 2048;

enum : int {
  kTotClosest = 0,
  kTotShadow,
  kTotNodes, kTotTris, kTotSph,
  kTotShNodes, kTotShPrims,
  kTotOverflow,
  kTotTail,
  kTotStackOverflow,
  kTotTracedP,
  kTotTracedB,
  kTotNodesP, kTotTrisP, kTotSphP,
  kTotTracedD,
  kTotNodesD = kTotTracedD + 8,
  kTotHistT = kTotNodesD + 8,
  kTotHistS = kTotHistT + 16,
  kTotHitP = kTotHistS + 16,
  kTotHitB,
  kTotStrag,
  kTotStragNodes, kTotStragTris, kTotStragSph,
  kTotTracedF,
  kTotWords
};

constexpr int kStatDepths = 8;
constexpr int kHistBins = 16;
static_assert(kTotWords == kTotTracedD + 8 + 8 + 16 + 16 + 7, "totals layout");

struct SegTable {
  uint32_t* cnt;
  uint32_t* per;
};

constexpr size_t kHitBytes = 12;
struct HitStream {
// ... 118 lines not shown
  sptr_frame frame;
  uint32_t k, tail;
  uint32_t chain, spare;
  uint32_t sky_split, sky_split_threads;
};
struct GraphCache {
  bool valid = false;
  GraphKey key{};
  DevGraph graph;
  DevGraphExec exec;
  hipGraphNode_t dyn_node = nullptr;
  hipKernelNodeParams dyn_params{};
  uint32_t waves = 0;
  uint32_t nodes = 0, edges = 0, depth = 0;
};

struct RefitState {
  bool valid = false;
  bool split = false;
  uint32_t num_verts = 0;
  DevBuf idx;
  DevBuf box_lo, box_hi;
  DevBuf order;
  DevBuf hoff;
  std::vector<uint32_t> hoff_h;
  uint32_t max_h = 0;
  DevBuf wsrc;
  DevBuf in_pos, in_sph;
  DevEvent ev[4];
  uint32_t refits = 0;
  double ms_wall = 0.0, ms_device = 0.0, ms_stage[3] = {0.0, 0.0, 0.0};
  DevBuf snap;
  DevEvent snap_ev[2];
  uint32_t snapshots = 0;
  double ms_snapshot = 0.0;
  bool xf_valid = false;
  DevBuf rest, in_xf;
  DevBuf cost_part;
  DevEvent cost_ev[2];
  double ms_cost = 0.0;
  double cost_upload = 0.0, area_upload = 0.0;
};

struct Context {
  int device = 0;
  DevStream stream;
  DevStream cap_stream;
  DevStream side_stream, cap_side, side2_stream, cap_side2;
  struct DepEvents {
    DevEvent fork, join, sky;
  } dev[2];
  int prio_lo = 0, prio_hi = 0;
  DevEvent quiet_ev[2];
  uint32_t launch_mode = 0;
  uint8_t* image_out = nullptr;
  const Context* parent = nullptr;
  bool last_forked = false;
  uint32_t strag_lanes = kStragLanesDefault;
  uint64_t epoch = 1;
  DevBuf dyn;
  DevBuf tslots;
  uint32_t tslots_used = 0;
  double wall_khz = 0.0;
  bool time_by_events = false;
  GraphCache graph;
  int32_t capture_status = 0;
  std::string capture_error;
  uint32_t captures = 0;
  GraphKey last_key{};
  bool have_last_key = false;
  GraphKey bad_key{};
  bool have_bad_key = false;
  std::string err;
  int debug_mode = 0;
  uint64_t wave_paths = 0;
  uint32_t tail_depth = 0;
  uint32_t bounce_chain = 0;
  uint32_t sky_split = 0;
  uint32_t sky_split_threads = 0;
  bool cull_listed = false;
  uint32_t sky_split_last = 0;
  DevBuf nodes, prim_ref, tris, sph, tri_geom, sph_geom, tri_orig, sph_orig, geom_mat;
  DevBuf tri_mat;
  uint32_t leaf_size = 0;
  uint32_t bvh_width = 0;
  uint32_t leaf_used = 0;
  uint32_t treelet_passes = SPTR_TREELET_PASSES;
  uint32_t num_nodes = 0, num_tris = 0, num_sph = 0, root = 0, bvh_depth = 0;
  uint32_t num_tri_refs = 0;
  uint32_t split_pieces = 1;
  uint32_t num_nodes4 = 0, root4 = 0;
  uint32_t excluded_prims = 0;
  uint32_t num_top4 = 0;
  uint32_t stack_need2 = 0, stack_need4 = 0;
  DevBuf nodes4;
  uint32_t num_tri_geoms = 0;
  std::vector<uint32_t> geom_first;
  std::vector<uint32_t> geom_material;
  bool have_scene = false;
  double build_ms = 0.0;
  bool dynamic = false;
  bool dynamic_xf = false;
  RefitState rf;
  std::vector<DevMaterial> mats_host;
  DevBuf mats;
  std::vector<DevLight> lights_host;
  DevBuf env;
  int32_t env_size = 0;
  float env_intensity = 0.8f, env_clamp = 5.0f;
  WaveBufs wb;
  DevBuf w_tot;
  int32_t W = 0, H = 0, G = 1, R = 0;
  uint32_t P = 0, local_tiles = 0;
  DevBuf accum, tiles, image;
  DevBuf cull;
  DevBuf plist;
  DevBuf entry;
  uint64_t cull_epoch = 0;
  sptr_camera cull_cam{};
  uint32_t cull_depth = 0;
  bool cull_exact = false;
  uint32_t last_samples = 0;
  uint32_t seed_offset = 0;
  DevBuf qbuf;
  std::vector<DevEvent> events;
  std::vector<StageMark> marks;
  size_t events_used = 0;
  uint32_t pending = 0;
  hipStream_t pending_stream = nullptr;
  uint64_t pending_samples = 0, pending_waves = 0, pending_culls = 0;
};

int build_lbvh(Context& c, const float* h_pos, uint32_t nverts, const uint32_t* h_idx, uint32_t ntris,
               const float* h_sph, uint32_t nsph, const uint32_t* h_tri_geom, uint32_t sph_geom_base);

int refit_retain_slots(Context& c, const float* d_pos, const uint32_t* d_idx, const float4* d_sph);
void launch_wide_sources(uint32_t ncur, const uint2* cur, uint32_t base, const BvhNode* nodes, uint32_t* wsrc, hipStream_t s);
int refit_lbvh(Context& c, const float* d_pos, const float4* d_sph, const float* d_xf = nullptr);
int refit_tree_cost(Context& c, double* cost, double* root_area);
int refit_snapshot(Context& c);
void refit_release(Context& c);

hipError_t scan_u32(void* temp, size_t& temp_bytes, const uint32_t* in, uint32_t* out, uint32_t n, hipStream_t s);
hipError_t radix_sort_pairs_u64(void* temp, size_t& temp_bytes, const uint64_t* keys_in, uint64_t* keys_out,
                                const uint32_t* vals_in, uint32_t* vals_out, uint32_t n, hipStream_t s);

SceneView scene_view(const Context& c);
unsigned launch_trace(const SceneView& sv, const ShadeView& sh, const FrameView& f, const WaveView& w, int depth, bool count,
                  uint32_t nseg_in, hipStream_t s);
bool shade_fuses_shadows(const SceneView& sv, const ShadeView& sh, bool count);
bool shadow_overlaps(const SceneView& sv, const WaveView& w);
unsigned launch_shade(const SceneView& sv, const ShadeView& sh, const FrameView& f, const WaveView& w, int depth,
                      uint32_t nseg, bool fuse, hipStream_t s);
unsigned launch_bounce01(const SceneView& sv, const ShadeView& sh, const FrameView& f, const WaveView& w, uint32_t nseg,
                         bool shade_first, bool close, hipStream_t s);
unsigned launch_bounce(const SceneView& sv, const ShadeView& sh, const FrameView& f, const WaveView& w, int depth,
                       uint32_t nseg, bool shade_first, bool close, hipStream_t s);
unsigned launch_bounce_chain(const SceneView& sv, const ShadeView& sh, const FrameView& f, const WaveView& w, int T,
                             uint32_t nseg, hipStream_t s);
unsigned launch_tail(const SceneView& sv, const ShadeView& sh, const FrameView& f, const WaveView& w, int depth0,
                     uint32_t nseg_in, hipStream_t s);
unsigned launch_shadow(const SceneView& sv, const ShadeView& sh, const WaveView& w, int depth, bool count, uint32_t nseg_in,
                   hipStream_t s);
void launch_strag(const SceneView& sv, const ShadeView& sh, const FrameView& f, const WaveView& w, int depth,
                  hipStream_t s);
bool trace_queue_applies(const SceneView& sv);
uint32_t hrec_mult(const SceneView& sv);
bool strag_applies(const SceneView& sv);
uint32_t bounce0_pixel_major(const SceneView& sv, const FrameView& f);
void launch_accumulate(const FrameView& f, const WaveView& w, float4* accum, uint32_t* tiles, uint8_t* image,
                       bool resolve, hipStream_t s);
uint32_t cull_depth_for(uint32_t spp, bool exact);
bool cull_entries_apply(const SceneView& sv);
void launch_cull(const SceneView& sv, const FrameView& f, uint32_t* mask, uint32_t* plist, uint32_t* entry, bool list_culled,
                 hipStream_t s);
void launch_sky(const ShadeView& sh, const FrameView& f, bool capped, hipStream_t s);
void launch_sky_list(const ShadeView& sh, const FrameView& f, hipStream_t s);
uint32_t sky_list_resident_threads(const ShadeView& sh);
void launch_interleave_tiles(const uint32_t* a, uint32_t na, const uint32_t* b, uint32_t nb, uint32_t* dst,
                             uint32_t n, hipStream_t s);
void launch_resolve(const FrameView& f, const float4* accum, uint32_t n, uint32_t* tiles, uint8_t* image,
                    hipStream_t s);
void launch_frame_dyn(uint32_t* dyn, uint32_t frame_begin, uint32_t reset, uint32_t total, uint32_t* clear,
                      unsigned long long* t0, hipStream_t s);
const void* frame_dyn_kernel();
void launch_pathtracer(const SceneView& sv, const ShadeView& sh, const FrameView& f, const WaveView& w, hipStream_t s);
void launch_optix(const SceneView& sv, const ShadeView& sh, const FrameView& f, const WaveView& w, hipStream_t s);
void launch_unpack(const uint32_t* gathered, int G, uint32_t tiles_per_rank, int W, int H, uint8_t* rgb,
                   hipStream_t s);
void launch_tri_materials(const uint32_t* tri_geom, const uint32_t* geom_mat, uint32_t n, uint32_t* tri_mat, hipStream_t s);
void launch_query(const SceneView& sv, const uint32_t* tri_orig, const uint32_t* sph_orig, const float* rays, uint32_t n,
                  bool anyhit, uint32_t* ref, float* t, float* ng, uint8_t* occ, uint32_t* stack_overflow, hipStream_t s);
void launch_primary(const FrameView& f, float* dirs, uint32_t* rng, hipStream_t s);
void launch_eval_math(int fn, const float* x, uint32_t n, float* out, hipStream_t s);
void launch_aov(const SceneView& sv, const FrameView& f, const AovView& a, hipStream_t s);
void launch_dn_mean(const DenoiseView& v, const float4* accum0, const float4* accum1, int G, float4* out, hipStream_t s);
void launch_atrous(const DenoiseView& v, const float4* cin, float4* cout, int step, float S2, hipStream_t s);
void launch_dn_resolve(const DenoiseView& v, const float4* c, uint8_t* image, hipStream_t s);
void launch_dn_reproject(const DenoiseView& v, const FrameView& f, const ReprojView& r, hipStream_t s);
void launch_dn_reproject_motion(const DenoiseView& v, const FrameView& f, const ReprojView& r, hipStream_t s);
void launch_atrous_history(const DenoiseView& v, const float4* cin, float4* cout, int step, float Si, hipStream_t s);
void launch_rayquery(const SceneView& sv, const RayQueryView& q, bool anyhit, hipStream_t s);
void launch_ray_keys(const SceneView& sv, const float4* rays, uint32_t n, uint64_t* keys, uint32_t* index, hipStream_t s);
void launch_spin(uint64_t ticks, hipStream_t s);

}
```

Measured before the change: 88110 Mrays/s.

## Precompute per-primitive material table and stage it in LDS for fused shading

Builds a flat per-primitive material-id table (triangles then spheres) at scene/material upload time and, in the fused shade/trace kernels, copies it into LDS after the staged scene. Surface lookup then reads the material id with one LDS or global word instead of a chained geom/tri_mat indirection, and reads the scene triangles and spheres from the staged LDS copy. Material records are loaded through explicit LDS-address-space word loads. This costs extra LDS per block, which may reduce occupancy, and fusion is now disabled when the table is absent.

```diff
diff --git a/simple-path-tracer_amd/csrc/kernels_wavefront.hip b/simple-path-tracer_amd/csrc/kernels_wavefront.hip
--- a/simple-path-tracer_amd/csrc/kernels_wavefront.hip
+++ b/simple-path-tracer_amd/csrc/kernels_wavefront.hip
@@ -796,10 +796,12 @@
   const uint32_t* prim_ref;
   const float4* tris;
   const float4* sph;
+  const uint32_t* pm;
+  bool pm_lds;
 };
 template <bool kLds>
 __device__ __forceinline__ Staged stage_scene(const SceneView& sv, float4* lds) {
-  Staged s{sv.nodes, sv.nodes4, sv.prim_ref, sv.tris, sv.sph};
+  Staged s{sv.nodes, sv.nodes4, sv.prim_ref, sv.tris, sv.sph, nullptr, false};
   if (kLds) {
     const bool w4 = sv.width == (uint32_t)kWide;
     const uint32_t nn = (w4 ? sv.num_nodes4 * (uint32_t)sizeof(WideNode) : sv.num_nodes * (uint32_t)sizeof(BvhNode)) / 16u,
@@ -817,6 +819,22 @@
     s.tris = lds + nn;
     s.sph = lds + nn + nt;
     s.prim_ref = reinterpret_cast<const uint32_t*>(lds + nn + nt + ns);
+  }
+  return s;
+}
+
+template <bool kTable>
+__device__ __forceinline__ Staged stage_shaded(const SceneView& sv, const ShadeView& sh, float4* lds) {
+  const bool tab = kTable && sh.pm_lds_bytes != 0u;
+  float4* dst = lds + sv.lds_bytes / 16u;
+  if (tab) {
+    const float4* g = reinterpret_cast<const float4*>(sh.prim_mat);
+    for (uint32_t i = threadIdx.x; i < sh.pm_lds_bytes / 16u; i += blockDim.x) dst[i] = g[i];
+  }
+  Staged s = stage_scene<true>(sv, lds);
+  if (kTable) {
+    s.pm = tab ? reinterpret_cast<const uint32_t*>(dst) : sh.prim_mat;
+    s.pm_lds = tab;
   }
   return s;
 }
@@ -1873,25 +1891,50 @@
   vec3 P, n;
   DevMaterial m;
 };
-__device__ __forceinline__ Surface surface_at(const SceneView& sv, const ShadeView& sh, const DevMaterial* smat,
-                                              uint32_t nm, vec3 ro, vec3 rd, float t, uint32_t ref) {
+typedef const uint32_t __attribute__((address_space(3))) * LdsWords;
+typedef const uint32_t __attribute__((address_space(1))) * GlobalWords;
+__device__ __forceinline__ uint32_t lds_word(const uint32_t* p) { return *(LdsWords)p; }
+__device__ __forceinline__ uint32_t global_word(const uint32_t* p) { return *(GlobalWords)p; }
+__device__ __forceinline__ DevMaterial lds_material(const DevMaterial* m) {
+  static_assert(sizeof(DevMaterial) == 12 * sizeof(uint32_t), "material words");
+  const uint32_t* w = reinterpret_cast<const uint32_t*>(m);
+  uint32_t v[12];
+#pragma unroll
+  for (int i = 0; i < 12; ++i) v[i] = lds_word(w + i);
+  DevMaterial out;
+  __builtin_memcpy(&out, v, sizeof(out));
+  return out;
+}
+enum ShadeFrom { kShadeGlobal = 0, kShadeFused = 1 };
+template <int kFrom>
+__device__ __forceinline__ Surface surface_at(const Staged& sc, const SceneView& sv, const ShadeView& sh,
+                                              const DevMaterial* smat, uint32_t nm, vec3 ro, vec3 rd, float t, uint32_t ref) {
   Surface s;
   s.P = ro + t * rd;
   const uint32_t idx = ref & kIndexMask;
+  const bool sphere = (ref & kSphereBit) != 0u;
+  const float4* sph = kFrom == kShadeGlobal ? sv.sph : sc.sph;
+  const float4* tris = kFrom == kShadeGlobal ? sv.tris : sc.tris;
   vec3 ng;
-  uint32_t mid;
-  if (ref & kSphereBit) {
-    const float4 c = sv.sph[idx];
+  uint32_t mid = 0u;
+  constexpr bool have_mid = kFrom == kShadeFused;
+  if constexpr (have_mid) {
+    const uint32_t pslot = prim_mat_slot(sv.num_tris, sphere, idx);
+    mid = sc.pm_lds ? lds_word(sc.pm + pslot) : global_word(sc.pm + pslot);
+  }
+  if (sphere) {
+    const float4 c = sph[idx];
     ng = v3((s.P.x - c.x) / c.w, (s.P.y - c.y) / c.w, (s.P.z - c.z) / c.w);
-    mid = sh.geom_mat[sv.sph_geom[idx]];
+    if (!have_mid) mid = sh.geom_mat[sv.sph_geom[idx]];
   } else {
-    const float4 c = sv.tris[3 * idx + 2];
+    const float4 c = tris[3 * idx + 2];
     ng = v3(c.y, c.z, c.w);
-    mid = sh.tri_mat ? sh.tri_mat[idx] : sh.geom_mat[sv.tri_geom[idx]];
+    if (!have_mid) mid = sh.tri_mat ? sh.tri_mat[idx] : sh.geom_mat[sv.tri_geom[idx]];
   }
   s.n = safe_normalize(ng);
   if (dot(s.n, rd) > 0.0f) s.n = -s.n;
-  s.m = (mid < nm) ? smat[mid] : sh.mats[mid];
+  if (kFrom != kShadeGlobal && sh.num_mats <= 32u) s.m = lds_material(smat + mid);
+  else s.m = (mid < nm) ? smat[mid] : sh.mats[mid];
   return s;
 }
 
@@ -2024,6 +2067,7 @@
     w.work[kWorkTraceQueue + threadIdx.x * 32u] = 0u;
   }
   const Staged sc = stage_scene<kFuse>(sv, lds);
+  constexpr int kFrom = kShadeGlobal;
   Visits vc;
   uint32_t rays = 0u;
   uint32_t per_in = 0u;
@@ -2070,7 +2114,7 @@
         radv = v3(1.0f, 1.0f, 1.0f);
         dirty = true;
       } else {
-        sf = surface_at(sv, sh, smat, nm, ro, rd, __uint_as_float(h.y), h.z);
+        sf = surface_at<kFrom>(sc, sv, sh, smat, nm, ro, rd, __uint_as_float(h.y), h.z);
         const vec3 emission = v3(sf.m.emission[0], sf.m.emission[1], sf.m.emission[2]);
         if (dot(emission, emission) > 0.0f) {
           if (!kPrimary) radv = xyz(w.rad[p]);
@@ -2160,7 +2204,7 @@
   }
 }
 
-template <bool kCube>
+template <bool kCube, int kFrom>
 __device__ __forceinline__ void bounce_ray(const Staged& sc, const SceneView& sv, const ShadeView& sh, const DevMaterial* smat,
                                            uint32_t nm, const WaveView& w, const RayStream& rin, const RayStream& rout,
                                            int depth, bool last, bool valid, uint32_t id, uint32_t seg0, uint32_t* s_cnt,
@@ -2188,7 +2232,7 @@
       radv = v3(1.0f, 1.0f, 1.0f);
       dirty = true;
     } else {
-      const Surface sf = surface_at(sv, sh, smat, nm, ro, rd, tfar, ref);
+      const Surface sf = surface_at<kFrom>(sc, sv, sh, smat, nm, ro, rd, tfar, ref);
       const vec3 emission = v3(sf.m.emission[0], sf.m.emission[1], sf.m.emission[2]);
       if (dot(emission, emission) > 0.0f) {
         radv = xyz(w.rad[p]) + thr * emission;
@@ -2226,13 +2270,14 @@
   if constexpr (kTimed) ktime_begin(w);
   const FrameView f = frame_dyn(fin);
   extern __shared__ float4 lds[];
-  uint32_t* s_off = reinterpret_cast<uint32_t*>(lds + sv.lds_bytes / 16u);
+  uint32_t* s_off = reinterpret_cast<uint32_t*>(lds + (sv.lds_bytes + sh.pm_lds_bytes) / 16u);
   __shared__ DevMaterial smat[32];
   __shared__ uint32_t s_cnt_n, s_rays;
   __shared__ LdsStack s_stack;
   const uint32_t nm = stage_materials(sh, smat);
   if (threadIdx.x == 0) s_cnt_n = s_rays = 0u;
-  const Staged sc = stage_scene<true>(sv, lds);
+  constexpr int kFrom = kShadeFused;
+  const Staged sc = stage_shaded<kFrom == kShadeFused>(sv, sh, lds);
   uint32_t per_in = 0u;
   const uint32_t n = seg_scan(w.segN, nseg_in, s_off, per_in);
   if (blockIdx.x == 0 && threadIdx.x == 0) {
@@ -2249,7 +2294,7 @@
     const uint32_t i = base + threadIdx.x;
     const bool valid = i < n;
     const uint32_t id = valid ? seg_slot(s_off, nseg_in, per_in, i) : 0u;
-    bounce_ray<kCube>(sc, sv, sh, smat, nm, w, rin, rout, depth, last, valid, id, sd.seg0, &s_cnt_n, vc, s_stack, rays);
+    bounce_ray<kCube, kFrom>(sc, sv, sh, smat, nm, w, rin, rout, depth, last, valid, id, sd.seg0, &s_cnt_n, vc, s_stack, rays);
   }
   for (int off = 32; off > 0; off >>= 1) rays += __shfl_xor(rays, off);
   if (lane_id() == 0u) atomicAdd(&s_rays, rays);
@@ -2263,7 +2308,7 @@
   if constexpr (kTimed) ktime_end(w);
 }
 
-template <bool kCube>
+template <bool kCube, int kFrom>
 __device__ __forceinline__ void bounce01_path(const Staged& sc, const SceneView& sv, const ShadeView& sh, const DevMaterial* smat,
                                               uint32_t nm, const FrameView& f, const ImageDiv& idiv, const WaveView& w,
                                               const RayStream& rout, bool last1, bool last2, bool valid, uint32_t slot,
@@ -2283,7 +2328,7 @@
       radv = v3(1.0f, 1.0f, 1.0f);
       active = false;
     } else {
-      const Surface sf = surface_at(sv, sh, smat, nm, f.cam_pos, pr.d, __uint_as_float(h.y), h.z);
+      const Surface sf = surface_at<kFrom>(sc, sv, sh, smat, nm, f.cam_pos, pr.d, __uint_as_float(h.y), h.z);
       const vec3 emission = v3(sf.m.emission[0], sf.m.emission[1], sf.m.emission[2]);
       if (dot(emission, emission) > 0.0f) radv = radv + thr * emission;
       vec3 so, ldir, contrib;
@@ -2307,7 +2352,7 @@
     if (!traverse_w<false, false, false>(sc, sv, make_ray(ro, rd), 0.0f, tfar, ref, vc, s_stack)) {
       radv = radv + thr * env_color<kCube>(sh.env, renormalized_again(rd));
     } else {
-      const Surface sf = surface_at(sv, sh, smat, nm, ro, rd, tfar, ref);
+      const Surface sf = surface_at<kFrom>(sc, sv, sh, smat, nm, ro, rd, tfar, ref);
       const vec3 emission = v3(sf.m.emission[0], sf.m.emission[1], sf.m.emission[2]);
       if (dot(emission, emission) > 0.0f) radv = radv + thr * emission;
       if (light_faces(sh.lights[0], sf)) lit = light_term(sh.lights[0], sf, -rd, thr, so, ldir, stfar, contrib);
@@ -2340,13 +2385,14 @@
   if constexpr (kTimed) ktime_begin(w);
   const FrameView f = frame_dyn(fin);
   extern __shared__ float4 lds[];
-  uint32_t* s_off = reinterpret_cast<uint32_t*>(lds + sv.lds_bytes / 16u);
+  uint32_t* s_off = reinterpret_cast<uint32_t*>(lds + (sv.lds_bytes + sh.pm_lds_bytes) / 16u);
   __shared__ DevMaterial smat[32];
   __shared__ uint32_t s_cnt_n, s_rays, s_traced;
   __shared__ LdsStack s_stack;
   const uint32_t nm = stage_materials(sh, smat);
   if (threadIdx.x == 0) s_cnt_n = s_rays = s_traced = 0u;
-  const Staged sc = stage_scene<true>(sv, lds);
+  constexpr int kFrom = kShadeFused;
+  const Staged sc = stage_shaded<kFrom == kShadeFused>(sv, sh, lds);
   uint32_t per_in = 0u;
   const uint32_t n = seg_scan(w.segH, nseg_in, s_off, per_in);
   const RayStream rout = w.rs[0];
@@ -2359,7 +2405,7 @@
     const uint32_t i = base + threadIdx.x;
     const bool valid = i < n;
     const uint32_t slot = valid ? seg_slot(s_off, nseg_in, per_in, i) : 0u;
-    bounce01_path<kCube>(sc, sv, sh, smat, nm, f, idiv, w, rout, last1, last2, valid, slot, sd.seg0, &s_cnt_n, vc, s_stack, rays,
+    bounce01_path<kCube, kFrom>(sc, sv, sh, smat, nm, f, idiv, w, rout, last1, last2, valid, slot, sd.seg0, &s_cnt_n, vc, s_stack, rays,
                          traced);
   }
   for (int off = 32; off > 0; off >>= 1) {
@@ -2392,13 +2438,14 @@
   if constexpr (kTimed) ktime_begin(w);
   const FrameView f = frame_dyn(fin);
   extern __shared__ float4 lds[];
-  uint32_t* s_off = reinterpret_cast<uint32_t*>(lds + sv.lds_bytes / 16u);
+  uint32_t* s_off = reinterpret_cast<uint32_t*>(lds + (sv.lds_bytes + sh.pm_lds_bytes) / 16u);
   __shared__ DevMaterial smat[32];
   __shared__ uint32_t s_cnt[3], s_rays, s_traced;
   __shared__ LdsStack s_stack;
   const uint32_t nm = stage_materials(sh, smat);
   if (threadIdx.x == 0) s_cnt[0] = s_cnt[1] = s_cnt[2] = s_rays = s_traced = 0u;
-  const Staged sc = stage_scene<true>(sv, lds);
+  constexpr int kFrom = kTimed ? kShadeGlobal : kShadeFused;
+  const Staged sc = stage_shaded<kFrom == kShadeFused>(sv, sh, lds);
   uint32_t per_in = 0u;
   const uint32_t n = seg_scan(w.segH, nseg_in, s_off, per_in);
   const bool last1 = 1u >= f.max_depth, last2 = 2u >= f.max_depth;
@@ -2412,7 +2459,7 @@
       const uint32_t i = base + threadIdx.x;
       const bool valid = i < n;
       const uint32_t slot = valid ? seg_slot(s_off, nseg_in, per_in, i) : 0u;
-      bounce01_path<kCube>(sc, sv, sh, smat, nm, f, idiv, w, rout, last1, last2, valid, slot, sd.seg0, &s_cnt[1], vc, s_stack,
+      bounce01_path<kCube, kFrom>(sc, sv, sh, smat, nm, f, idiv, w, rout, last1, last2, valid, slot, sd.seg0, &s_cnt[1], vc, s_stack,
                            rays, traced);
     }
   }
@@ -2430,7 +2477,7 @@
     for (uint32_t j = 0u; j < cnt; j += kBlock) {
       const uint32_t id = sd.seg0 + j + threadIdx.x;
       const bool valid = j + threadIdx.x < cnt && id < w.seg_cap;
-      bounce_ray<kCube>(sc, sv, sh, smat, nm, w, rin, rout, d, last, valid, id, sd.seg0, &s_cnt[d % 3], vc, s_stack, rays);
+      bounce_ray<kCube, kFrom>(sc, sv, sh, smat, nm, w, rin, rout, d, last, valid, id, sd.seg0, &s_cnt[d % 3], vc, s_stack, rays);
     }
   }
   for (int off = 32; off > 0; off >>= 1) {
@@ -2478,7 +2525,7 @@
   if (!traverse_w<false, true, false>(sc, sv, make_ray(so, ldir), 1e-4f, stfar, sref, vc, s_stack))
     rad_add(w, p, dirty, radv, contrib);
 }
-template <bool kCube, bool kFirst, bool kClose>
+template <bool kCube, bool kFirst, bool kClose, int kFrom>
 __device__ __forceinline__ void shade_trace(const Staged& sc, const SceneView& sv, const ShadeView& sh, const DevMaterial* smat,
                                             uint32_t nm, const FrameView& f, const ImageDiv& idiv, const WaveView& w,
                                             const RayStream& rin, const RayStream& rout, int depth, bool last, bool valid,
@@ -2515,7 +2562,7 @@
       radv = v3(1.0f, 1.0f, 1.0f);
       dirty = true;
     } else {
-      const Surface sf = surface_at(sv, sh, smat, nm, ro, rd, t, ref);
+      const Surface sf = surface_at<kFrom>(sc, sv, sh, smat, nm, ro, rd, t, ref);
       const vec3 emission = v3(sf.m.emission[0], sf.m.emission[1], sf.m.emission[2]);
       if (dot(emission, emission) > 0.0f) rad_add(w, p, dirty, radv, thr * emission);
       if (light_faces(sh.lights[0], sf)) lit = light_term(sh.lights[0], sf, -rd, thr, so, ldir, stfar, contrib);
@@ -2548,7 +2595,7 @@
     vec3 no2, nd2;
     lit = false;
     if (hit) {
-      const Surface sf = surface_at(sv, sh, smat, nm, no, nd, tfar, href);
+      const Surface sf = surface_at<kFrom>(sc, sv, sh, smat, nm, no, nd, tfar, href);
       const vec3 emission = v3(sf.m.emission[0], sf.m.emission[1], sf.m.emission[2]);
       if (dot(emission, emission) > 0.0f) rad_add(w, p, dirty, radv, thr * emission);
       if (light_faces(sh.lights[0], sf)) lit = light_term(sh.lights[0], sf, -nd, thr, so, ldir, stfar, contrib);
@@ -2575,13 +2622,14 @@
   if constexpr (kTimed) ktime_begin(w);
   const FrameView f = frame_dyn(fin);
   extern __shared__ float4 lds[];
-  uint32_t* s_off = reinterpret_cast<uint32_t*>(lds + sv.lds_bytes / 16u);
+  uint32_t* s_off = reinterpret_cast<uint32_t*>(lds + (sv.lds_bytes + sh.pm_lds_bytes) / 16u);
   __shared__ DevMaterial smat[32];
   __shared__ uint32_t s_cnt_n, s_rays, s_traced;
   __shared__ LdsStack s_stack;
   const uint32_t nm = stage_materials(sh, smat);
   if (threadIdx.x == 0) s_cnt_n = s_rays = s_traced = 0u;
-  const Staged sc = stage_scene<true>(sv, lds);
+  constexpr int kFrom = (kTimed && kCube && !kFirst && !kClose) ? kShadeGlobal : kShadeFused;
+  const Staged sc = stage_shaded<kFrom == kShadeFused>(sv, sh, lds);
   const SegTable tin = kFirst ? w.segH : w.segN, tout = kFirst ? w.segN : w.segH;
   uint32_t per_in = 0u;
   const uint32_t n = seg_scan(tin, nseg_in, s_off, per_in);
@@ -2595,7 +2643,7 @@
     const uint32_t i = base + threadIdx.x;
     const bool valid = i < n;
     const uint32_t slot = valid ? seg_slot(s_off, nseg_in, per_in, i) : 0u;
-    shade_trace<kCube, kFirst, kClose>(sc, sv, sh, smat, nm, f, idiv, w, rin, rout, depth, last, valid, slot, sd.seg0, &s_cnt_n,
+    shade_trace<kCube, kFirst, kClose, kFrom>(sc, sv, sh, smat, nm, f, idiv, w, rin, rout, depth, last, valid, slot, sd.seg0, &s_cnt_n,
                                        vc, s_stack, rays, traced);
   }
   for (int off = 32; off > 0; off >>= 1) {
@@ -2777,6 +2825,7 @@
   if (threadIdx.x < 2u) s_rays[threadIdx.x] = 0u;
   if (threadIdx.x == 0u) s_next = 0u;
   const Staged sc = stage_scene<kLds>(sv, lds);
+  constexpr int kFrom = kShadeGlobal;
   const uint32_t ntop = (walk_reads_top(kWalkU) && kW4 && !kLds) ? sv.num_top4 : 0u;
   const uint4* top = ntop ? stage_top(sv, lds + top_lds_offset(sv, kLds, false, nseg_in)) : nullptr;
   uint32_t per_in = 0u;
@@ -2846,7 +2895,7 @@
         radv = radv + thr * env_color<kCube>(sh.env, renormalized_again(rd));
         break;
       }
-      const Surface sf = surface_at(sv, sh, smat, nm, ro, rd, tfar, ref);
+      const Surface sf = surface_at<kFrom>(sc, sv, sh, smat, nm, ro, rd, tfar, ref);
       const vec3 emission = v3(sf.m.emission[0], sf.m.emission[1], sf.m.emission[2]);
       if (dot(emission, emission) > 0.0f) radv = radv + thr * emission;
       const vec3 view = -rd;
@@ -2899,6 +2948,7 @@
   if (threadIdx.x < 2u) s_rays[threadIdx.x] = 0u;
   if (threadIdx.x == 0u) s_next = 0u;
   const Staged sc = stage_scene<false>(sv, nullptr);
+  constexpr int kFrom = kShadeGlobal;
   extern __shared__ float4 lds[];
   const uint32_t ntop = walk_reads_top(kWalkU) ? sv.num_top4 : 0u;
   const uint4* top = ntop ? stage_top(sv, lds) : nullptr;
@@ -2973,7 +3023,7 @@
         radv = radv + thr * env_color<kCube>(sh.env, renormalized_again(rd));
         break;
       }
-      const Surface sf = surface_at(sv, sh, smat, nm, ro, rd, tfar, ref);
+      const Surface sf = surface_at<kFrom>(sc, sv, sh, smat, nm, ro, rd, tfar, ref);
       const vec3 emission = v3(sf.m.emission[0], sf.m.emission[1], sf.m.emission[2]);
       if (dot(emission, emission) > 0.0f) radv = radv + thr * emission;
       const vec3 view = -rd;
@@ -3869,7 +3919,7 @@
 #ifdef SPTR_EXPERIMENT_KNOBS
   if (getenv("SPTR_NO_FUSE")) return false;
 #endif
-  return sv.lds_bytes != 0 && sv.width == 2u && sh.num_lights == 1u && !count;
+  return sv.lds_bytes != 0 && sv.width == 2u && sh.num_lights == 1u && !count && sh.prim_mat != nullptr;
 }
 
 unsigned launch_shade(const SceneView& sv, const ShadeView& sh, const FrameView& f, const WaveView& w, int depth,
@@ -3903,7 +3953,7 @@
 unsigned launch_bounce(const SceneView& sv, const ShadeView& sh, const FrameView& f, const WaveView& w_in, int depth,
                        uint32_t nseg, bool shade_first, bool close, hipStream_t s) {
   const WaveView w = with_tslot(w_in);
-  const unsigned lb = sv.lds_bytes + (4u * (nseg + 1u) + 15u) / 16u * 16u;
+  const unsigned lb = sv.lds_bytes + sh.pm_lds_bytes + (4u * (nseg + 1u) + 15u) / 16u * 16u;
   if (!shade_first)
     return dispatch(
         [&](auto fl) -> unsigned {
@@ -3928,7 +3978,7 @@
 unsigned launch_bounce01(const SceneView& sv, const ShadeView& sh, const FrameView& f, const WaveView& w_in, uint32_t nseg,
                          bool shade_first, bool close, hipStream_t s) {
   const WaveView w = with_tslot(w_in);
-  const unsigned lb = sv.lds_bytes + (4u * (nseg + 1u) + 15u) / 16u * 16u;
+  const unsigned lb = sv.lds_bytes + sh.pm_lds_bytes + (4u * (nseg + 1u) + 15u) / 16u * 16u;
   if (!shade_first)
     return dispatch(
         [&](auto fl) -> unsigned {
@@ -3953,7 +4003,7 @@
 unsigned launch_bounce_chain(const SceneView& sv, const ShadeView& sh, const FrameView& f, const WaveView& w_in, int T,
                              uint32_t nseg, hipStream_t s) {
   const WaveView w = with_tslot(w_in);
-  const unsigned lb = sv.lds_bytes + (4u * (nseg + 1u) + 15u) / 16u * 16u;
+  const unsigned lb = sv.lds_bytes + sh.pm_lds_bytes + (4u * (nseg + 1u) + 15u) / 16u * 16u;
   return dispatch(
       [&](auto fl) -> unsigned {
         return [&]<bool Cube, bool Tm>(Flags<Cube, Tm>) {
@@ -4141,6 +4191,20 @@
   if (n) hipLaunchKernelGGL(k_tri_materials, dim3(grid_for(n)), dim3(kBlock), 0, s, tri_geom, geom_mat, n, tri_mat);
 }
 
+__global__ void __launch_bounds__(kBlock) k_prim_materials(const uint32_t* tri_geom, const uint32_t* sph_geom,
+                                                           const uint32_t* geom_mat, uint32_t num_tris, uint32_t num_sph,
+                                                           uint32_t* prim_mat) {
+  const uint32_t n = prim_mat_bytes(num_tris, num_sph) / 4u;
+  for (uint32_t i = blockIdx.x * blockDim.x + threadIdx.x; i < n; i += grid_threads())
+    prim_mat[i] = prim_mat_entry(tri_geom, sph_geom, geom_mat, num_tris, num_sph, i);
+}
+void launch_prim_materials(const uint32_t* tri_geom, const uint32_t* sph_geom, const uint32_t* geom_mat, uint32_t num_tris,
+                           uint32_t num_sph, uint32_t* prim_mat, hipStream_t s) {
+  const uint32_t n = prim_mat_bytes(num_tris, num_sph) / 4u;
+  if (n) hipLaunchKernelGGL(k_prim_materials, dim3(grid_for(n)), dim3(kBlock), 0, s, tri_geom, sph_geom, geom_mat, num_tris,
+                            num_sph, prim_mat);
+}
+
 void launch_unpack(const uint32_t* gathered, int G, uint32_t tiles_per_rank, int W, int H, uint8_t* rgb,
                    hipStream_t s) {
   const int ntx = (W + kTile - 1) / kTile;
diff --git a/simple-path-tracer_amd/csrc/prim_mat_table.h b/simple-path-tracer_amd/csrc/prim_mat_table.h
--- /dev/null
+++ b/simple-path-tracer_amd/csrc/prim_mat_table.h
@@ -0,0 +1,29 @@
+#pragma once
+#include <stdint.h>
+
+#if defined(__HIPCC__)
+#define SPTR_PM __host__ __device__ __forceinline__
+#else
+#define SPTR_PM inline
+#endif
+
+namespace sptr {
+
+SPTR_PM uint32_t prim_mat_entries(uint32_t num_tris, uint32_t num_sph) { return num_tris + num_sph; }
+SPTR_PM uint32_t prim_mat_bytes(uint32_t num_tris, uint32_t num_sph) {
+  return (prim_mat_entries(num_tris, num_sph) * 4u + 15u) / 16u * 16u;
+}
+SPTR_PM uint32_t prim_mat_slot(uint32_t num_tris, bool sphere, uint32_t idx) { return sphere ? num_tris + idx : idx; }
+SPTR_PM uint32_t prim_mat_entry(const uint32_t* tri_geom, const uint32_t* sph_geom, const uint32_t* geom_mat,
+                                uint32_t num_tris, uint32_t num_sph, uint32_t i) {
+  if (i < num_tris) return geom_mat[tri_geom[i]];
+  if (i < num_tris + num_sph) return geom_mat[sph_geom[i - num_tris]];
+  return 0u;
+}
+SPTR_PM uint32_t prim_mat_lds_bytes(uint32_t scene_lds_bytes, uint32_t num_tris, uint32_t num_sph, uint32_t cap) {
+  const uint32_t tb = prim_mat_bytes(num_tris, num_sph);
+  if (scene_lds_bytes == 0u || prim_mat_entries(num_tris, num_sph) == 0u) return 0u;
+  return scene_lds_bytes + tb <= cap ? tb : 0u;
+}
+
+}
diff --git a/simple-path-tracer_amd/csrc/sptr_api.cpp b/simple-path-tracer_amd/csrc/sptr_api.cpp
--- a/simple-path-tracer_amd/csrc/sptr_api.cpp
+++ b/simple-path-tracer_amd/csrc/sptr_api.cpp
@@ -158,9 +158,28 @@
 constexpr uint64_t kShadeFirstMinPaths = SPTR_SHADE_FIRST_MIN_PATHS;
 bool shade_first_on(uint64_t batch_paths) { return batch_paths > kShadeFirstMinPaths; }
 
+int build_prim_materials(Context& c) {
+  const Context& own = shading(c);
+  c.prim_mat_n = 0u;
+  const uint32_t n = prim_mat_entries(c.num_tri_refs, c.num_sph);
+  if (!c.have_scene || n == 0u || own.mats_host.empty() || own.geom_mat.p == nullptr ||
+      own.num_tri_geoms != c.num_tri_geoms || own.num_sph != c.num_sph || scene_view(c).lds_bytes == 0u)
+    return SPTR_OK;
+  API_HIP(hipSetDevice(c.device));
+  API_HIP(c.prim_mat.ensure(prim_mat_bytes(c.num_tri_refs, c.num_sph)));
+  launch_prim_materials(static_cast<const uint32_t*>(c.tri_geom.p), static_cast<const uint32_t*>(c.sph_geom.p),
+                        static_cast<const uint32_t*>(own.geom_mat.p), c.num_tri_refs, c.num_sph,
+                        static_cast<uint32_t*>(c.prim_mat.p), c.stream);
+  API_HIP(hipGetLastError());
+  API_HIP(hipStreamSynchronize(c.stream));
+  c.prim_mat_n = n;
+  return SPTR_OK;
+}
+
 int resolve_geom_materials(Context& c) {
   const uint32_t nm = (uint32_t)c.mats_host.size();
   const uint32_t ng = c.num_tri_geoms + c.num_sph;
+  c.prim_mat_n = 0u;
   if (!c.have_scene || nm == 0) return SPTR_OK;
   std::vector<uint32_t> t(ng ? ng : 1, 0u);
   for (uint32_t g = 0; g < ng; ++g) {
@@ -182,7 +201,7 @@
     API_HIP(hipGetLastError());
     API_HIP(hipStreamSynchronize(c.stream));
   }
-  return SPTR_OK;
+  return build_prim_materials(c);
 }
 
 inline bool host_local_pixel(const Context& c, uint32_t l, int& x, int& y) {
@@ -323,6 +342,9 @@
   s.num_mats = (uint32_t)c.mats_host.size();
   s.geom_mat = static_cast<const uint32_t*>(c.geom_mat.p);
   s.tri_mat = cc.parent ? nullptr : static_cast<const uint32_t*>(c.tri_mat.p);
+  const bool pm = cc.prim_mat_n != 0u && cc.prim_mat_n == prim_mat_entries(cc.num_tri_refs, cc.num_sph);
+  s.prim_mat = pm ? static_cast<const uint32_t*>(cc.prim_mat.p) : nullptr;
+  s.pm_lds_bytes = pm ? prim_mat_lds_bytes(scene_view(cc).lds_bytes, cc.num_tri_refs, cc.num_sph, kLdsSceneBytes) : 0u;
   s.num_lights = (uint32_t)c.lights_host.size();
   for (uint32_t i = 0; i < s.num_lights; ++i) s.lights[i] = c.lights_host[i];
   s.env.env = static_cast<const float4*>(c.env.p);
@@ -1298,7 +1320,7 @@
     return fail(x->c, SPTR_ERR_INVALID, "bvh width must be 0 (auto), 2 or " + std::to_string(kWide));
   x->c.bvh_width = width;
   ++x->c.epoch;
-  return SPTR_OK;
+  return build_prim_materials(x->c);
 }
 
 static int set_tail_depth_one(sptr_ctx* x, uint32_t depth) {
@@ -1370,6 +1392,7 @@
     for (uint32_t i = s->tri_geom_first[g]; i < s->tri_geom_first[g + 1]; ++i) tg[i] = g;
   }
   c.have_scene = false;
+  c.prim_mat_n = 0u;
   c.num_tri_geoms = s->num_tri_geoms;
   c.geom_first.assign(s->tri_geom_first, s->tri_geom_first + (s->num_tri_geoms ? s->num_tri_geoms + 1 : 0));
   c.geom_material.assign(s->geom_material, s->geom_material + s->num_tri_geoms + s->num_spheres);
@@ -2163,6 +2186,8 @@
     const int r1 = upload_scene_one(x->lane, s);
     if (r1 != SPTR_OK) return lane_forward(x, r1);
     x->lane_scene = true;
+    const int r2 = build_prim_materials(cy);
+    if (r2 != SPTR_OK) return lane_forward(x, r2);
   }
   return SPTR_OK;
 }
@@ -2968,7 +2993,13 @@
 int sptr_set_materials(sptr_ctx* x, const sptr_material* m, uint32_t n) {
   const int rs = lane_shading_sync(x);
   if (rs != SPTR_OK) return rs;
-  return lane_shading_changed(x, set_materials_one(x, m, n));
+  const int rc = lane_shading_changed(x, set_materials_one(x, m, n));
+  if (rc != SPTR_OK || !x->lane) return rc;
+  if (!x->lane_scene) {
+    x->lane->c.prim_mat_n = 0u;
+    return rc;
+  }
+  return lane_forward(x, build_prim_materials(x->lane->c));
 }
 
 int sptr_set_lights(sptr_ctx* x, const sptr_light* l, uint32_t n) {
diff --git a/simple-path-tracer_amd/csrc/sptr_internal.h b/simple-path-tracer_amd/csrc/sptr_internal.h
--- a/simple-path-tracer_amd/csrc/sptr_internal.h
+++ b/simple-path-tracer_amd/csrc/sptr_internal.h
@@ -6,6 +6,7 @@
 #include <vector>
 
 #include "dev_owned.h"
+#include "prim_mat_table.h"
 #include "sptr_hip.h"
 #include "sptr_math.h"
 #include "tile_map.h"
@@ -105,6 +106,8 @@
   DevLight lights[kMaxLights];
   EnvView env;
   int32_t debug_mode;
+  const uint32_t* prim_mat;
+  uint32_t pm_lds_bytes;
 };
 
 struct FrameView {
@@ -389,6 +392,8 @@
   uint32_t sky_split_last = 0;
   DevBuf nodes, prim_ref, tris, sph, tri_geom, sph_geom, tri_orig, sph_orig, geom_mat;
   DevBuf tri_mat;
+  DevBuf prim_mat;
+  uint32_t prim_mat_n = 0;
   uint32_t leaf_size = 0;
   uint32_t bvh_width = 0;
   uint32_t leaf_used = 0;
@@ -496,6 +501,8 @@
 void launch_unpack(const uint32_t* gathered, int G, uint32_t tiles_per_rank, int W, int H, uint8_t* rgb,
                    hipStream_t s);
 void launch_tri_materials(const uint32_t* tri_geom, const uint32_t* geom_mat, uint32_t n, uint32_t* tri_mat, hipStream_t s);
+void launch_prim_materials(const uint32_t* tri_geom, const uint32_t* sph_geom, const uint32_t* geom_mat, uint32_t num_tris,
+                           uint32_t num_sph, uint32_t* prim_mat, hipStream_t s);
 void launch_query(const SceneView& sv, const uint32_t* tri_orig, const uint32_t* sph_orig, const float* rays, uint32_t n,
                   bool anyhit, uint32_t* ref, float* t, float* ng, uint8_t* occ, uint32_t* stack_overflow, hipStream_t s);
 void launch_primary(const FrameView& f, float* dirs, uint32_t* rng, hipStream_t s);
```

New measurement: 90320 Mrays/s (median of 6 runs). +2.5%, better.
